# AntonioFerreras/Digital-Earth

Hardware: AMD Instinct MI355X
Metric: Msamples/sec (1920x1080, 64 spp) spectral path tracing (higher is better)
Workload: dtype f32; 1 GPU; 1920x1080, 64 spp, full spectral Rayleigh+Mie+O3+clouds, quality-2 synthetic maps, default camera, BASELINE configs[1]; parallelism=single GPU, frames_in_flight=1, launch_slots=3, waves_per_cu=24, primed_frames=4, kernel=per-CU stage scheduler, launches_per_call=1

## Files before the change

### digital_earth_amd/build.py

```python
import os
import subprocess

_HERE = os.path.dirname(os.path.abspath(__file__))
CSRC = os.path.join(_HERE, "csrc")
OUT = os.path.join(_HERE, "libdigitalearth_hip.so")
OUT_LEGACY = os.path.join(_HERE, "libdigitalearth_hip_legacy.so")
SOURCES = ["de_api.hip", "de_fast.hip"]
DEPS = ["de_api.hip", "de_fast.hip", "de_rccl.h", "de_launch.h", "de_host_consts.h", "de_context.h", "render_kernel.hip", "render_kernel_v2.hip", "de_stages.h", "render_kernel_v6.hip",
        "aux_kernels.hip", "adaptive_kernels.hip", "denoise_kernels.hip", "exposure_kernels.hip", "bloom_kernels.hip", "history_kernels.hip", "pixels_kernels.hip", "local_exposure_kernels.hip", "output_scale_kernels.hip", "hdr_output_kernels.hip", "de_kernels.h", "de_device.h", "de_math.h", os.path.join("..", "..", "include", "digital_earth.h"),
        os.path.join("..", "..", "include", "digital_earth_debug.h"), os.path.join("..", "..", "include", "digital_earth_denoise.h"),
        os.path.join("..", "..", "include", "digital_earth_exposure.h"), os.path.join("..", "..", "include", "digital_earth_bloom.h"),
        os.path.join("..", "..", "include", "digital_earth_history.h"), os.path.join("..", "..", "include", "digital_earth_pixels.h"),
        os.path.join("..", "..", "include", "digital_earth_local_exposure.h"), os.path.join("..", "..", "include", "digital_earth_output_scale.h"),
        os.path.join("..", "..", "include", "digital_earth_hdr_output.h")]
DEPS_LEGACY = DEPS + [os.path.join("legacy", f) for f in ("render_kernel_v3.hip", "render_kernel_v5.hip", "de_launch_legacy.h", "de_ctx_legacy_members.inc")]
FLAGS = ["--offload-arch=gfx950", "-O3", "-std=c++17", "-ffp-contract=off", "-fno-fast-math", "-fno-slp-vectorize", "-fPIC",
         "-shared", "-Wno-unused-value", "-mllvm", "-enable-ipra", "-fno-optimize-sibling-calls"]


def needs_build():
    if not os.path.exists(OUT):
        return True
    t = os.path.getmtime(OUT)
    return any(os.path.getmtime(os.path.join(CSRC, d)) > t for d in DEPS)


def build(force=False, verbose=False):
    if not force and not needs_build():
        return OUT
    hipcc = os.environ.get("HIPCC", "/opt/rocm/bin/hipcc")
    extra = os.environ.get("DE_EXTRA_FLAGS", "").split()
    cmd = [hipcc] + FLAGS + extra + [os.path.join(CSRC, s) for s in SOURCES] + ["-o", OUT]
    if verbose:
        print(" ".join(cmd))
    subprocess.check_call(cmd, cwd=CSRC)
    return OUT


def build_legacy(force=False, verbose=False):
    if not force and os.path.exists(OUT_LEGACY) and all(os.path.getmtime(os.path.join(CSRC, d)) <= os.path.getmtime(OUT_LEGACY) for d in DEPS_LEGACY):
        return OUT_LEGACY
    hipcc = os.environ.get("HIPCC", "/opt/rocm/bin/hipcc")
    cmd = [hipcc] + FLAGS + ["-DDE_LEGACY_VARIANTS"] + os.environ.get("DE_EXTRA_FLAGS", "").split() + [os.path.join(CSRC, s) for s in SOURCES] + ["-o", OUT_LEGACY]
    if verbose:
        print(" ".join(cmd))
    subprocess.check_call(cmd, cwd=CSRC)
    return OUT_LEGACY


TEST_VARIANTS = (("v6_p64", ["-DDE_V6_P=64u", "-DDE_V6_CAP=65u"]), ("v6_p128", ["-DDE_V6_P=128u", "-DDE_V6_CAP=129u"]), ("v6_cap_p1", ["-DDE_V6_CAP=1121u"]),
                 ("v6_no_cloud_bound", ["-DDE_NO_CLOUD_BOUND"]))


def build_test_variants(force=False, verbose=False):
    root = os.path.dirname(_HERE)
    out_dir = os.path.join(root, "build", "ab")
    os.makedirs(out_dir, exist_ok=True)
    hipcc = os.environ.get("HIPCC", "/opt/rocm/bin/hipcc")
    newest = max(os.path.getmtime(os.path.join(CSRC, d)) for d in DEPS)
    procs = []
    for name, flags in TEST_VARIANTS:
        out = os.path.join(out_dir, name + ".so")
        if not force and os.path.exists(out) and os.path.getmtime(out) >= newest:
            continue
        cmd = [hipcc] + FLAGS + flags + [os.path.join(CSRC, s) for s in SOURCES] + ["-o", out]
        if verbose:
            print(" ".join(cmd))
        procs.append((name, subprocess.Popen(cmd, cwd=CSRC)))
    for name, pr in procs:
        if pr.wait() != 0:
            raise RuntimeError("building the test variant %s failed" % name)


if __name__ == "__main__":
    build(force=True, verbose=True)
```

### digital_earth_amd/csrc/de_context.h

```cpp
#pragma once
#include "de_kernels.h"
#include "../../include/digital_earth_exposure.h"
#include "../../include/digital_earth_bloom.h"
#include "../../include/digital_earth_history.h"
#include "../../include/digital_earth_pixels.h"
#include "../../include/digital_earth_local_exposure.h"
#include "../../include/digital_earth_output_scale.h"
#include "../../include/digital_earth_hdr_output.h"

#include <dlfcn.h>
#include <math.h>
#include <stdio.h>
#include <stdlib.h>
#include <string.h>
#include <mutex>
#include <string>
#include <vector>

#include "render_kernel.hip"
#include "render_kernel_v2.hip"
#include "de_stages.h"
#ifdef DE_LEGACY_VARIANTS
#include "legacy/render_kernel_v3.hip"
#include "legacy/render_kernel_v5.hip"
#endif
#include "render_kernel_v6.hip"
#include "aux_kernels.hip"
#include "adaptive_kernels.hip"
#include "denoise_kernels.hip"
#include "exposure_kernels.hip"
#include "bloom_kernels.hip"
#include "history_kernels.hip"
#include "pixels_kernels.hip"
#include "output_scale_kernels.hip"
#include "local_exposure_kernels.hip"
#include "hdr_output_kernels.hip"

namespace {

#define DE_N_COUNTERS 64
thread_local std::string g_err;
int fail(int code, const std::string& msg) { g_err = msg; return code; }

#define HIP_TRY(expr)                                                                                   \
    do {                                                                                                \
        hipError_t e_ = (expr);                                                                         \
        if (e_ != hipSuccess) return fail(DE_ERR_HIP, std::string(#expr) + ": " + hipGetErrorString(e_)); \
    } while (0)

enum { DE_FRAME_NONE = 0, DE_FRAME_UNIFORM = 1, DE_FRAME_ADAPTIVE = 2 };

#define DE_MAX_SLOTS 8
#define DE_FETCH_RING 4
struct LaunchSlot {
    hipStream_t stream = nullptr;
    hipEvent_t done = nullptr;
    hipEvent_t t0 = nullptr, t1 = nullptr;
    uint2* contrib = nullptr;
    size_t contrib_items = 0;
    bool pending = false;
    bool launched = false;
    uint64_t seen_render = 0, seen_hdr = 0;
};

struct DevTexture {
    int w = 0, h = 0, ch = 0;
    uint8_t* linear = nullptr;
    uint32_t* packed = nullptr;
    int tiles_x = 0, tiles_y = 0;
    int packed_clamp = -1;
    uint8_t* bound = nullptr;
    bool set = false;
    bool borrowed = false;
};

}

struct de_ctx {
    int device = 0;
    int W = 0, H = 0;
    de_params p;
    bool params_dirty = true;
    bool nodes_dirty = true;
    int tune_pend = 18, tune_heavy = 13, tune_b = 24, tune_gas = 6, tune_chunk = 128, tune_wpc = 20, tune_max_spp = 0;
    hipStream_t stream = nullptr;
    bool own_stream = false;
    LaunchSlot slot[DE_MAX_SLOTS];
    int n_slots = 8, big_slots = 3, next_slot = 0, last_slot = -1;
    int last_v6_slot = -1;
    int cu_withhold = 0;
    float* d_standin = nullptr;
    hipEvent_t ev_standin[16][2] = {};
    unsigned standin_count = 0;
    bool last_reduce_standin = false;
    hipEvent_t ev_main = nullptr;
    uint64_t gen_render = 1, gen_hdr = 1, rec_render = 0, rec_hdr = 0;
    int t0_slot = -1, t1_slot = -1;
    bool timing_valid = false;
    bool timing_empty = false;
    DevTexture tex[DE_TEX_COUNT];
    float* d_cie = nullptr;
    float* d_srgb2spec = nullptr;
    float* d_o3 = nullptr;
    float* d_crf = nullptr;
    int n_crf = 0;
    bool luts_set = false;
    bool luts_borrowed = false;
    FrameConsts* d_fc = nullptr;
    LambdaNode* d_nodes = nullptr;
    float* d_node_val = nullptr;
    float* d_hdr = nullptr;
    float* d_hdr_own = nullptr;
    float* d_image = nullptr;
    float* d_scratch = nullptr;
    float* h_stage = nullptr;
    size_t h_stage_bytes = 0;
    float* h_ring[DE_FETCH_RING] = {};
    size_t h_ring_bytes[DE_FETCH_RING] = {};
    hipEvent_t ev_ring[DE_FETCH_RING] = {};
    unsigned fetch_begun = 0, fetch_ended = 0;
    uint32_t* d_tiles = nullptr;
    int n_tiles = 0, tiles_rank = -1, tiles_world = -1;
    unsigned long long* d_counters = nullptr;
    uint32_t* d_work_counter = nullptr;
    float* d_dens_table = nullptr;
    int n_cus = 256;
    bool count = false;
    de_counters counters;
    int current_spp = 0;
    int sample_rank = 0, sample_world = 1;
    float* d_assembled = nullptr;
    float* d_gather = nullptr;
    int gather_world = 0;
    const float* display_src = nullptr;
    hipEvent_t ev_r0 = nullptr, ev_r1 = nullptr;
    bool reduce_timing_valid = false;
    void* comm = nullptr;
    int comm_rank = 0, comm_world = 1;
    bool trace = false;
    int kernel_variant = 4;
    struct V6State {
        wf::Cold* cold = nullptr;
        uint32_t* ctl = nullptr;
        RenderArgs* d_args = nullptr;
        uint32_t* h_status = nullptr;
        uint32_t n_wg = 0;
        uint4* pool[2] = {nullptr, nullptr};
        uint32_t pool_cap[2] = {0, 0};
    } v6s[DE_MAX_SLOTS];
    int v6_tail_levels = 1, v6_tail_export[2] = {128, 96}, v6_tail_grid[2] = {64, 8};
    uint32_t v6_tail_min_paths = 4u << 20;
    int v6_tail_when_alone = 0;
    uint32_t* h_issued = nullptr;
    uint32_t v6_launch_seq = 0;
    int v6_bands = 8;
    int v6_stats = 0;
    int v6_svc[3] = {24, 24, 20};
    int v6_svc_area[3] = {100, 72, 90};
    int v6_yield = 56, v6_elsewhere = 48, v6_retry = 6, v6_enter_min = 0, v6_flat_min = 0, v6_flat_again = 32;
    int launch_variant = 2;
    int launch_pipe = 0;
    int launch_slot = 0;
    bool launch_one_batch = false;
    int last_call[4] = {0, 0, 0, 0};
    int launch_pipes = 1;
    int launch_depths = 25, launch_wpc = 14;
    int auto_v6 = 1;
    unsigned long long auto_v6_min_items = 1ull << 12;
    size_t mem_budget = 0;
#ifdef DE_LEGACY_VARIANTS
#include "legacy/de_ctx_legacy_members.inc"
#endif
    int frame_kind = 0;
    float* d_s2 = nullptr;
    uint32_t* d_alist[2] = {nullptr, nullptr};
    int32_t* d_tile_spp = nullptr;
    uint32_t* d_keep = nullptr;
    int32_t* d_ad_count = nullptr;
    int32_t* h_ad_count = nullptr;
    int ad_cur = 0, ad_active = 0, ad_n = 0, ad_rounds = 0;
    unsigned long long ad_pixel_samples = 0;
    uint64_t ad_seed = 0;
    float ad_threshold = 0.f, ad_floor = 0.f;
    int ad_min = 0, ad_max = 0, ad_round = 0;
    bool dn_on = false;
    int dn_levels = 5;
    float dn_sigma_l = 4.0f;
    bool dn_s2_complete = false;
    bool dn_guides_valid = false;
    bool dn_out_valid = false;
    float4* d_dn_nc = nullptr;
    float4* d_dn_at = nullptr;
    float* d_dn_dist = nullptr;
    float4* d_dn_buf[2] = {nullptr, nullptr};
    float* d_dn_out = nullptr;
    bool ae_on = false;
    bool ae_displayed = false;
    de_auto_exposure ae;
    uint32_t* d_ae_partial = nullptr;
    double* d_ae_centre = nullptr;
    MeterState* d_ae_state = nullptr;
    FrameConsts* d_fc_ae = nullptr;
    MeterResult* d_ae_result = nullptr;
    bool bl_on = false;
    de_bloom bl;
    float4* d_bl_pyr = nullptr;
    float* d_bl_out = nullptr;
    bool hs_on = false;
    bool hs_valid = false;
    bool hs_cand_valid = false;
    de_history hs;
    float4* d_hs_c[2] = {nullptr, nullptr};
    float* d_hs_d[2] = {nullptr, nullptr};
    HistoryCam* d_hs_cam[2] = {nullptr, nullptr};
    int hs_cur = 0;
    float* d_hs_out = nullptr;
    de_pixels px = {(uint32_t)sizeof(de_pixels), 4, DE_PIXELS_TRUNCATE, 0u, 0};
    uint32_t px_count = 0;
    uint32_t px_last_phase = 0;
    uint8_t* d_px = nullptr;
    uint8_t* h_px_stage = nullptr;
    uint8_t* h_px_ring[DE_FETCH_RING] = {};
    hipEvent_t ev_px_ring[DE_FETCH_RING] = {};
    unsigned px_begun = 0, px_ended = 0;
    size_t d_px_bytes = 0, h_px_stage_bytes = 0, h_px_ring_bytes[DE_FETCH_RING] = {};
    bool lx_on = false;
    de_local_exposure lx;
    float2* d_lx_pyr = nullptr;
    float* d_lx_base = nullptr;
    float* d_lx_out = nullptr;
    de_output_scale os = {(uint32_t)sizeof(de_output_scale), 0, 0, 0, DE_SCALE_LANCZOS3};
    struct ScaleDev {
        int32_t* first = nullptr;
        float* w = nullptr;
        size_t first_cap = 0, w_cap = 0;
        int n_src = 0, n_dst = 0, filter = -1, taps = 0;
    } os_tab[2];
    float* d_os_mid = nullptr;
    float* d_os_out = nullptr;
    size_t os_mid_bytes = 0, os_out_bytes = 0;
    de_hdr_output ho = {(uint32_t)sizeof(de_hdr_output), 0, 1000.0f, DE_HDR_GAMUT_REC2020, DE_HDR_TRANSFER_PQ, DE_HDR_PIXELS_RGB10A2, DE_PIXELS_TRUNCATE, 0u, 0};
    HdrConsts ho_consts = {};
    uint32_t ho_count = 0;
    uint32_t ho_last_phase = 0;
    void* d_hpx = nullptr;
    uint8_t* h_hpx_stage = nullptr;
    size_t d_hpx_bytes = 0, h_hpx_stage_bytes = 0;
    bool frame_invalid = false;
    std::string invalid_msg;
    de_ctx* lender = nullptr;
    int loans = 0;
};
```

### digital_earth_amd/csrc/de_kernels.h

```cpp
#pragma once
#include "de_device.h"
#include "../../include/digital_earth_debug.h"

struct FrameConsts {
    vec3 cam_pos, d, du, dv;
    float fov, aspect_ratio, aspect_scale;
    vec3 light_dir;
    vec3 sun_x, sun_y;
    float sun_cos_angle, sun_angular_radius;
    float land_height_scale;
    float normal_eps;
    float offset_scale;
    float kn_log;
    float max_dens_r, max_dens_m, max_dens_o;
    CloudPhaseConsts cloud;
    float exposure_scale;
    float gamma;
    float crf_slice_v;
    float vig_strength, vig_radius, vig_cx, vig_cy;
    float drt_m, drt_s, drt_fl, drt_ds, drt_clamp_max, drt_dch_s;
    vec3 drt_w;
    float agx_srgb_to_xyz[9], agx_xyz_to_adjusted[9];
    float agx_x_pivot, agx_y_pivot, agx_toe_scale, agx_shoulder_scale;
    int use_agx;
};

struct LambdaNode {
    float wavelength;
    float rx, ry, rz;
    float rcp_pdf;
    float ext_r, ext_m, ext_o;
    float sun_power, night_power, sun_irradiance;
    float max_ext_rmo;
    float c0, c1, c2;
    float s2s_valid;
    float inv_max_ext_rmo;
    float pad0, pad1, pad2;
};
#define DE_N_NODES 512
#ifndef DE_DENS_TABLE_N
#define DE_DENS_TABLE_N 262144
#endif
#ifndef DE_DENS_STRIDE
#define DE_DENS_STRIDE 3
#endif

struct RenderArgs {
    const FrameConsts* fc;
    const LambdaNode* nodes;
    const float* node_val;
    const float* dens_table;
    TexR8 topo, ocean, clouds, bathy, emissive;
    TexRGB albedo, stars;
    float* hdr;
    int W, H;
    const uint32_t* tiles;
    int n_tiles, tiles_x;
    int tiles_identity;
    uint32_t seed_lo, seed_hi;
    int spp_begin, spp_count;
    int spp_stride;
    int fixed_wavelength;
    unsigned long long* counters;
    float* debug_out;
    uint32_t* work_counter;
    unsigned long long spp_magic;
    uint2* contrib;
    int pend_thr;
    int heavy_thr;
    int chunk;
    int gas_thr;
    int tune_b;
    const uint4* resume_rec;
    const uint32_t* resume_count;
    const float* resume_cold;
    uint32_t resume_capacity;
    const uint8_t* cloud_bound;
};

#ifndef DE_CLOUD_BOUND_N
#define DE_CLOUD_BOUND_N 128
#endif
#ifndef DE_CLOUD_BOUND_R
#define DE_CLOUD_BOUND_R 24576u
#endif
#define DE_CLOUD_BOUND_BYTES (6u * DE_CLOUD_BOUND_N * DE_CLOUD_BOUND_N)
DE_DEV uint32_t cloud_bound_cell(float x, float y, float z) {
    const float ax = de_abs(x), ay = de_abs(y), az = de_abs(z);
    float s, t, m;
    uint32_t f;
    if (ax >= ay && ax >= az) { f = x < 0.0f ? 1u : 0u; s = y; t = z; m = ax; }
    else if (ay >= az) { f = y < 0.0f ? 3u : 2u; s = x; t = z; m = ay; }
    else { f = z < 0.0f ? 5u : 4u; s = x; t = y; m = az; }
    const float r = __builtin_amdgcn_rcpf(m);
    const float hn = (float)(DE_CLOUD_BOUND_N / 2);
    const int i = (int)((s * r + 1.0f) * hn), j = (int)((t * r + 1.0f) * hn);
    const uint32_t ic = (uint32_t)min(max(i, 0), DE_CLOUD_BOUND_N - 1), jc = (uint32_t)min(max(j, 0), DE_CLOUD_BOUND_N - 1);
    return (f * (uint32_t)DE_CLOUD_BOUND_N + jc) * (uint32_t)DE_CLOUD_BOUND_N + ic;
}

struct SetupArgs {
    de_params p;
    int W, H;
    int topo_w;
    int n_crf;
    TexF3 cie;
    const float* srgb2spec;
    const float* o3;
    float drt[6];
    float agx[22];
    FrameConsts* fc;
    LambdaNode* nodes;
    float* node_val;
    int do_nodes;
};

struct DisplayArgs {
    const FrameConsts* fc;
    const float* hdr;
    float* image;
    TexF3 crf;
    int W, H, samples, clamp;
    const int32_t* tile_spp;
};
```

### digital_earth_amd/csrc/de_launch.h

```cpp
#pragma once
#include "de_host_consts.h"

namespace {


int join_slots(de_ctx* c) {
    for (int i = 0; i < c->n_slots; ++i) {
        LaunchSlot& s = c->slot[i];
        if (!s.pending) continue;
        HIP_TRY(hipStreamWaitEvent(c->stream, s.done, 0));
        s.pending = false;
    }
    return DE_OK;
}
bool launches_in_flight(de_ctx* c) {
    bool busy = false;
    for (int i = 0; i < c->n_slots && !busy; ++i)
        if (c->slot[i].launched && hipEventQuery(c->slot[i].done) == hipErrorNotReady) busy = true;
    (void)hipGetLastError();
    return busy;
}
void touched_render_inputs(de_ctx* c) { c->gen_render++; }
void touched_hdr(de_ctx* c) { c->gen_hdr++; }
void note_abort(de_ctx* c);
int frame_status(de_ctx* c);
int sync_all(de_ctx* c) {
    for (int i = 0; i < c->n_slots; ++i)
        if (c->slot[i].stream) HIP_TRY(hipStreamSynchronize(c->slot[i].stream));
    for (int i = 0; i < c->n_slots; ++i) c->slot[i].pending = false;
    HIP_TRY(hipStreamSynchronize(c->stream));
    note_abort(c);
    return DE_OK;
}
void release_loan(de_ctx* c) {
    if (c->lender) { c->lender->loans--; c->lender = nullptr; }
}

int build_cloud_bound(de_ctx* c, DevTexture& t) {
    if (!t.bound) HIP_TRY(hipMalloc(&t.bound, DE_CLOUD_BOUND_BYTES));
    uint8_t* tiles = nullptr;
    HIP_TRY(hipMalloc(&tiles, (size_t)t.tiles_x * t.tiles_y));
    hipLaunchKernelGGL(tile_max_kernel, dim3((unsigned)((t.tiles_x + 255) / 256), (unsigned)t.tiles_y), dim3(256), 0, c->stream, t.packed, tiles, t.w, t.h, t.tiles_x, t.tiles_y);
    hipError_t e = hipGetLastError();
    if (e == hipSuccess) {
        hipLaunchKernelGGL(cloud_bound_kernel, dim3(DE_CLOUD_BOUND_BYTES), dim3(64), 0, c->stream, tiles, t.bound, t.w, t.h, t.tiles_x, t.tiles_y, 1.5 * (double)DE_CLOUD_BOUND_R + 64.0);
        e = hipGetLastError();
    }
    if (e == hipSuccess) e = hipStreamSynchronize(c->stream);
    if (e != hipSuccess) (void)hipStreamSynchronize(c->stream);
    hipFree(tiles);
    if (e != hipSuccess) return fail(DE_ERR_HIP, std::string("building the cloud map's occupancy bound: ") + hipGetErrorString(e));
    return DE_OK;
}

int ensure_packed(de_ctx* c, int slot, bool clamp) {
    DevTexture& t = c->tex[slot];
    if (t.packed_clamp == (clamp ? 1 : 0)) return DE_OK;
    if (t.borrowed) return fail(DE_ERR_STATE, "a shared texture keeps its owner's address mode: set DE_FLAG_CLAMP_SAMPLER on the owner and render there once, then share again");
    if (!t.linear) return fail(DE_ERR_STATE, "the sampler address mode cannot change after de_trim_textures released the as-uploaded maps: upload or generate them again");
    if (c->loans > 0 && t.packed_clamp != -1) return fail(DE_ERR_STATE, "the maps are lent to another context (de_share_textures): they cannot be repacked for another address mode until every borrower is destroyed or holds maps of its own");
    { int rc = join_slots(c); if (rc) return rc; }
    touched_render_inputs(c);
    if (t.ch == 1) {
        dim3 grid((unsigned)((t.w + 255) / 256), (unsigned)t.h);
        hipLaunchKernelGGL(pack_r8_kernel, grid, dim3(256), 0, c->stream, t.linear, t.packed, t.w, t.h, t.tiles_x, clamp ? 1 : 0);
        if (slot == DE_TEX_CLOUDS) { HIP_TRY(hipGetLastError()); int rc = build_cloud_bound(c, t); if (rc) return rc; }
    } else {
        size_t n = (size_t)t.w * t.h;
        hipLaunchKernelGGL(pack_rgb_kernel, dim3((unsigned)((n + 255) / 256)), dim3(256), 0, c->stream, t.linear, t.packed, n);
    }
    HIP_TRY(hipGetLastError());
    t.packed_clamp = clamp ? 1 : 0;
    return DE_OK;
}

int alloc_texture(de_ctx* c, int slot, int w, int h, int ch) {
    DevTexture& t = c->tex[slot];
    if ((unsigned long long)(ch == 1 ? ((w + 7) / 8) * 8 : w) * (unsigned long long)(ch == 1 ? ((h + 3) / 4) * 4 : h) >= (1ull << 30))
        return fail(DE_ERR_INVALID, "map too large: the packed copy (one dword per texel) must stay below 4 GB — the kernels address it with a 32-bit byte offset");
    if (c->loans > 0) return fail(DE_ERR_STATE, "the maps are lent to another context (de_share_textures): destroy the borrowers, or give them maps of their own, before replacing a map");
    { int rc = sync_all(c); if (rc) return rc; }
    if (t.linear && !t.borrowed) hipFree(t.linear);
    if (t.packed && !t.borrowed) hipFree(t.packed);
    if (t.bound && !t.borrowed) hipFree(t.bound);
    t.linear = nullptr; t.packed = nullptr; t.bound = nullptr; t.borrowed = false;
    {
        bool any = false;
        for (int i = 0; i < DE_TEX_COUNT; ++i) any = any || (i != slot && c->tex[i].borrowed);
        if (!any && !c->luts_borrowed) release_loan(c);
    }
    touched_render_inputs(c);
    t.w = w; t.h = h; t.ch = ch; t.set = false; t.packed_clamp = -1;
    HIP_TRY(hipMalloc(&t.linear, (size_t)w * h * ch));
    if (ch == 1) {
        t.tiles_x = (w + 7) / 8; t.tiles_y = (h + 3) / 4;
        HIP_TRY(hipMalloc(&t.packed, (size_t)t.tiles_x * t.tiles_y * 32 * sizeof(uint32_t)));
    } else {
        t.tiles_x = t.tiles_y = 0;
        HIP_TRY(hipMalloc(&t.packed, (size_t)w * h * sizeof(uint32_t)));
    }
    return DE_OK;
}

int run_setup(de_ctx* c) {
    if (!c->params_dirty && !c->nodes_dirty) return DE_OK;
    { int rc = join_slots(c); if (rc) return rc; }
    touched_render_inputs(c);
    SetupArgs s;
    s.p = c->p;
    opendrt_consts(&s.drt[0], &s.drt[1], &s.drt[2], &s.drt[3], &s.drt[4], &s.drt[5]);
    agx_consts(s.agx);
    s.W = c->W; s.H = c->H;
    s.topo_w = c->tex[DE_TEX_TOPOGRAPHY].w > 0 ? c->tex[DE_TEX_TOPOGRAPHY].w : 1;
    s.n_crf = c->n_crf;
    s.cie.data = c->d_cie; s.cie.w = 441; s.cie.h = 2;
    s.srgb2spec = c->d_srgb2spec; s.o3 = c->d_o3;
    s.fc = c->d_fc; s.nodes = c->d_nodes; s.node_val = c->d_node_val;
    s.do_nodes = c->nodes_dirty ? 1 : 0;
    hipLaunchKernelGGL(setup_kernel, dim3(c->nodes_dirty ? DE_N_NODES / 64 : 1), dim3(64), 0, c->stream, s);
    HIP_TRY(hipGetLastError());
    c->params_dirty = false; c->nodes_dirty = false;
    return DE_OK;
}

int build_tiles(de_ctx* c, int rank, int world) {
    if (c->tiles_rank == rank && c->tiles_world == world && c->d_tiles) return DE_OK;
    { int rc = sync_all(c); if (rc) return rc; }
    touched_render_inputs(c);
    const int tx = c->W / 8, ty = c->H / 8;
    std::vector<uint32_t> tiles;
    tiles.reserve((size_t)tx * ty / world + tx);
    for (int y = 0; y < ty; ++y)
        for (int x = 0; x < tx; ++x)
            if (world <= 1 || ((x + y) % world) == rank) tiles.push_back((uint32_t)(y * tx + x));
    if (!c->d_tiles) HIP_TRY(hipMalloc(&c->d_tiles, (size_t)tx * ty * sizeof(uint32_t)));
    if (!tiles.empty()) HIP_TRY(hipMemcpyAsync(c->d_tiles, tiles.data(), tiles.size() * sizeof(uint32_t), hipMemcpyHostToDevice, c->stream));
    HIP_TRY(hipStreamSynchronize(c->stream));
    c->n_tiles = (int)tiles.size(); c->tiles_rank = rank; c->tiles_world = world;
    return DE_OK;
}

int fill_render_args(de_ctx* c, RenderArgs* a) {
    for (int i = 0; i < DE_TEX_COUNT; ++i)
        if (!c->tex[i].set) return fail(DE_ERR_STATE, "all 7 textures must be uploaded or generated before rendering");
    if (!c->luts_set) return fail(DE_ERR_STATE, "LUTs must be uploaded before rendering");
    const bool clamp = (c->p.flags & DE_FLAG_CLAMP_SAMPLER) != 0;
    for (int i = 0; i < DE_TEX_COUNT; ++i) { int rc = ensure_packed(c, i, clamp); if (rc) return rc; }
    int rc = run_setup(c);
    if (rc) return rc;
    auto r8 = [&](int slot) {
        const DevTexture& t = c->tex[slot];
        TexR8 o; o.data = t.packed; o.w = t.w; o.h = t.h; o.tiles_x = t.tiles_x; o.wf = (float)t.w; o.hf = (float)t.h;
        return o;
    };
    auto rgb = [&](int slot) {
        const DevTexture& t = c->tex[slot];
        TexRGB o; o.data = t.packed; o.w = t.w; o.h = t.h; o.wf = (float)t.w; o.hf = (float)t.h;
        return o;
    };
    a->fc = c->d_fc; a->nodes = c->d_nodes; a->node_val = c->d_node_val; a->dens_table = c->d_dens_table;
    a->topo = r8(DE_TEX_TOPOGRAPHY); a->ocean = r8(DE_TEX_OCEAN); a->clouds = r8(DE_TEX_CLOUDS);
    a->bathy = r8(DE_TEX_BATHYMETRY); a->emissive = r8(DE_TEX_EMISSIVE);
    a->albedo = rgb(DE_TEX_ALBEDO); a->stars = rgb(DE_TEX_STARS);
    a->hdr = c->d_hdr; a->W = c->W; a->H = c->H;
    a->tiles = c->d_tiles; a->n_tiles = c->n_tiles; a->tiles_x = c->W / 8; a->tiles_identity = (c->tiles_world <= 1) ? 1 : 0;
    a->fixed_wavelength = (c->p.flags & DE_FLAG_FIXED_WAVELENGTH) ? 1 : 0;
    a->counters = c->d_counters; a->debug_out = c->d_scratch; a->work_counter = c->d_work_counter;
    a->resume_rec = nullptr; a->resume_count = nullptr; a->resume_cold = nullptr; a->resume_capacity = 0;
    a->cloud_bound = c->tex[DE_TEX_CLOUDS].bound;
    a->pend_thr = c->tune_pend; a->heavy_thr = c->tune_heavy; a->tune_b = c->tune_b; a->gas_thr = c->tune_gas; a->chunk = c->tune_chunk;
    return DE_OK;
}

#ifdef DE_LEGACY_VARIANTS
hipError_t launch_v3(de_ctx* c, const RenderArgs& a, hipStream_t stream, int pipe);
hipError_t launch_v5(de_ctx* c, const RenderArgs& a, hipStream_t stream, int idx, const uint4* resume_rec = nullptr, const uint32_t* resume_count = nullptr,
                     const float* resume_cold = nullptr, uint32_t resume_capacity = 0, int wpc = 0);
void legacy_note_abort(de_ctx* c);
#endif

int v6_reserve(de_ctx* c, int idx, hipStream_t stream, unsigned long long n_items) {
    de_ctx::V6State& S = c->v6s[idx];
    const uint32_t n_wg = (uint32_t)(c->cu_withhold > 0 ? c->n_cus - 8 * c->cu_withhold : c->n_cus) * DE_V6_WG_PER_CU;
    uint32_t want[2] = {0u, 0u};
    const bool tail = n_items >= (unsigned long long)c->v6_tail_min_paths;
    if (tail && c->v6_tail_levels >= 1) want[0] = n_wg * (uint32_t)c->v6_tail_export[0];
    if (tail && c->v6_tail_levels >= 2) want[1] = std::min((uint32_t)c->v6_tail_grid[0], n_wg) * (uint32_t)c->v6_tail_export[1];
    for (int k = 0; k < 2; ++k) {
        if (S.pool_cap[k] >= want[k]) continue;
        HIP_TRY(hipStreamSynchronize(stream));
        if (S.pool[k]) hipFree(S.pool[k]);
        S.pool[k] = nullptr; S.pool_cap[k] = 0;
        if (hipMalloc(&S.pool[k], (size_t)want[k] * DE_V6_POOL_ENTRY_BYTES + 64u) != hipSuccess) { (void)hipGetLastError(); S.pool[k] = nullptr; return fail(DE_ERR_NOMEM, "no room for the tail pool of a render_kernel_v6 launch slot"); }
        S.pool_cap[k] = want[k];
    }
    if (S.cold && S.ctl && S.d_args && S.h_status && S.n_wg == n_wg) return DE_OK;
    HIP_TRY(hipStreamSynchronize(stream));
    if (S.cold) hipFree(S.cold);
    S.cold = nullptr; S.n_wg = 0;
    if (hipMalloc(&S.cold, (size_t)n_wg * DE_V6_P * sizeof(wf::Cold)) != hipSuccess) { (void)hipGetLastError(); S.cold = nullptr; return fail(DE_ERR_NOMEM, "no room for the cold records of a render_kernel_v6 launch slot (37 MB)"); }
    S.n_wg = n_wg;
    if (!S.ctl) HIP_TRY(hipMalloc(&S.ctl, (size_t)bs::G_WORDS * DE_V6_CTL_STRIDE * sizeof(uint32_t)));
    if (!S.d_args) HIP_TRY(hipMalloc(&S.d_args, sizeof(RenderArgs)));
    if (!S.h_status) {
        HIP_TRY(hipHostMalloc(reinterpret_cast<void**>(&S.h_status), 64, hipHostMallocMapped));
        S.h_status[0] = 0u;
    }
    return DE_OK;
}
}
hipError_t de_fast_launch_v6(const bs::Args& A, const FrameConsts* fc, dim3 grid, dim3 block, hipStream_t stream, bool clamp, bool tail);
namespace {
hipError_t launch_v6(de_ctx* c, const RenderArgs& a, hipStream_t stream, int idx) {
    de_ctx::V6State& S = c->v6s[idx];
    const bool clamp = (c->p.flags & DE_FLAG_CLAMP_SAMPLER) != 0;
    bs::Args A;
    A.ra = S.d_args; A.cold = S.cold; A.ctl = S.ctl;
    uint32_t* d_status = nullptr;
    hipError_t e = hipHostGetDevicePointer(reinterpret_cast<void**>(&d_status), S.h_status, 0);
    if (e != hipSuccess) return e;
    A.status = d_status;
    A.n_items = (uint32_t)((size_t)a.n_tiles * 64u * (size_t)a.spp_count);
    A.idle_limit = 1u << 22;
    for (int k = 0; k < 3; ++k) { A.svc[k] = (uint32_t)c->v6_svc[k]; A.svc_area[k] = (uint32_t)c->v6_svc_area[k]; }
    A.yield_max = (uint32_t)c->v6_yield; A.elsewhere_min = (uint32_t)c->v6_elsewhere; A.retry = (uint32_t)c->v6_retry; A.enter_min = (uint32_t)c->v6_enter_min; A.flat_min = (uint32_t)c->v6_flat_min; A.flat_again = (uint32_t)(c->v6_flat_again > 0 ? c->v6_flat_again : 1);
    A.bands = c->v6_bands == 8 ? 8u : 1u;
    hipLaunchKernelGGL(v6_init_kernel, dim3(1), dim3(256), 0, stream, S.ctl, a, S.d_args);
    const unsigned by_work = (unsigned)((A.n_items + 64u * DE_V6_WAVES - 1u) / (64u * DE_V6_WAVES));
    dim3 grid(by_work < S.n_wg ? (by_work ? by_work : 1u) : S.n_wg), block(64 * DE_V6_WAVES);
    const int levels = A.n_items >= c->v6_tail_min_paths ? c->v6_tail_levels : 0;
    if (!c->h_issued) {
        e = hipHostMalloc(reinterpret_cast<void**>(&c->h_issued), 64, hipHostMallocMapped);
        if (e != hipSuccess) return e;
        c->h_issued[0] = 0u;
    }
    uint32_t* d_issued = nullptr;
    e = hipHostGetDevicePointer(reinterpret_cast<void**>(&d_issued), c->h_issued, 0);
    if (e != hipSuccess) return e;
    const uint32_t seq = ++c->v6_launch_seq;
    if (c->last_v6_slot >= 0 && c->last_v6_slot != idx) __atomic_store_n(c->h_issued, seq - 1u, __ATOMIC_RELEASE);
    c->last_v6_slot = idx;
    A.issued = d_issued; A.seq = c->v6_tail_when_alone ? 0xffffffffu : seq;
    const bool fast = (c->p.flags & DE_FLAG_FAST_MATH) != 0u;
    for (int l = 0; l <= levels; ++l) {
        A.level = (uint32_t)l;
        A.export_at = l < levels ? (uint32_t)c->v6_tail_export[l] : 0u;
        A.pool_out = l < levels ? S.pool[l & 1] : nullptr; A.cap_out = l < levels ? S.pool_cap[l & 1] : 0u;
        A.pool_in = l > 0 ? S.pool[(l - 1) & 1] : nullptr; A.cap_in = l > 0 ? S.pool_cap[(l - 1) & 1] : 0u;
        const dim3 g = l == 0 ? grid : dim3(std::min((unsigned)c->v6_tail_grid[l - 1], (unsigned)S.n_wg));
        if (fast) { hipError_t e2 = de_fast_launch_v6(A, a.fc, g, block, stream, clamp, l > 0); if (e2 != hipSuccess) return e2; continue; }
        if (l == 0) {
            if (c->v6_stats && !clamp) hipLaunchKernelGGL((v6_kernel<false, true, false>), g, block, 0, stream, A, a.fc);
            else if (clamp) hipLaunchKernelGGL((v6_kernel<true, false, false>), g, block, 0, stream, A, a.fc);
            else hipLaunchKernelGGL((v6_kernel<false, false, false>), g, block, 0, stream, A, a.fc);
        } else {
            if (c->v6_stats && !clamp) hipLaunchKernelGGL((v6_kernel<false, true, true>), g, block, 0, stream, A, a.fc);
            else if (clamp) hipLaunchKernelGGL((v6_kernel<true, false, true>), g, block, 0, stream, A, a.fc);
            else hipLaunchKernelGGL((v6_kernel<false, false, true>), g, block, 0, stream, A, a.fc);
        }
    }
    return hipGetLastError();
}
void note_abort(de_ctx* c) {
    for (int i = 0; i < DE_MAX_SLOTS; ++i) {
        de_ctx::V6State& S = c->v6s[i];
        if (S.h_status && S.h_status[0] != 0u) {
            const uint32_t code = S.h_status[0];
            S.h_status[0] = 0u;
            c->frame_invalid = true;
            c->invalid_msg = std::string("render_kernel_v6 left on its abort word (") + (code == bs::ERR_ENTRY_TIMEOUT ? "a ring entry was never stored" : code == bs::ERR_CELL_BUSY_TIMEOUT ? "a ring cell was never emptied" : code == bs::ERR_POOL_FULL ? "the tail pool overflowed" : "idle watchdog: work was lost") + "): the frame is invalid until de_reset";
        }
    }
#ifdef DE_LEGACY_VARIANTS
    legacy_note_abort(c);
#endif
}
int frame_status(de_ctx* c) {
    note_abort(c);
    return c->frame_invalid ? fail(DE_ERR_HIP, c->invalid_msg) : DE_OK;
}

hipError_t launch_accumulate(de_ctx* c, const RenderArgs& a, dim3 grid, dim3 block, hipStream_t stream) {
    if (c->frame_kind == DE_FRAME_ADAPTIVE || (c->dn_on && c->dn_s2_complete)) hipLaunchKernelGGL(accumulate_moments_kernel, grid, block, 0, stream, a, c->d_s2);
    else hipLaunchKernelGGL(accumulate_kernel, grid, block, 0, stream, a);
    return hipGetLastError();
}

template <int MODE, typename PreAcc>
hipError_t launch_render(de_ctx* c, const RenderArgs& a, hipStream_t stream, PreAcc pre_acc) {
    const bool clamp = (c->p.flags & DE_FLAG_CLAMP_SAMPLER) != 0;
    const bool march = (c->p.flags & DE_FLAG_RAY_MARCHER) != 0;
    dim3 grid((unsigned)((a.n_tiles + 3) / 4)), block(256);
#ifdef DE_LEGACY_VARIANTS
    if (!march && (c->launch_variant == 5 || c->launch_variant == 3) && MODE == 0) {
        hipError_t el = c->launch_variant == 5 ? launch_v5(c, a, stream, c->launch_slot) : launch_v3(c, a, stream, c->launch_pipe);
        if (el != hipSuccess) return el;
        hipError_t pe = pre_acc();
        if (pe != hipSuccess) return pe;
        return launch_accumulate(c, a, grid, block, stream);
    }
#endif
    if (!march && c->launch_variant == 6 && MODE == 0) {
        hipError_t e6 = launch_v6(c, a, stream, c->launch_slot);
        if (e6 != hipSuccess) return e6;
        hipError_t pe = pre_acc();
        if (pe != hipSuccess) return pe;
        return launch_accumulate(c, a, grid, block, stream);
    }
    if (!march && c->launch_variant != 1) {
        hipError_t me = hipMemsetAsync(a.work_counter, 0, sizeof(uint32_t), stream);
        if (me != hipSuccess) return me;
        const unsigned waves_per_block = DE_V2_BLOCK / 64;
        const unsigned waves_per_cu = (unsigned)c->tune_wpc;
        const unsigned max_waves = (unsigned)c->n_cus * waves_per_cu;
        const unsigned long long items = (unsigned long long)a.n_tiles * 64ull * (unsigned long long)a.spp_count;
        const unsigned long long by_work = (items + (unsigned long long)a.chunk - 1ull) / (unsigned long long)a.chunk;
        const unsigned n_waves = by_work >= (unsigned long long)max_waves ? max_waves : (unsigned)(by_work > 0 ? by_work : 1ull);
        dim3 pgrid((n_waves + waves_per_block - 1) / waves_per_block), pblock(DE_V2_BLOCK);
        if (clamp) hipLaunchKernelGGL((render_kernel_v2<true, MODE>), pgrid, pblock, 0, stream, a, a.fc);
        else hipLaunchKernelGGL((render_kernel_v2<false, MODE>), pgrid, pblock, 0, stream, a, a.fc);
        if (MODE != 2) {
            hipError_t pe = pre_acc();
            if (pe != hipSuccess) return pe;
            return launch_accumulate(c, a, grid, block, stream);
        }
        return hipGetLastError();
    }
    hipError_t pe = pre_acc();
    if (pe != hipSuccess) return pe;
    if (march) {
        if (clamp) hipLaunchKernelGGL((ray_march_kernel<true, MODE>), grid, block, 0, stream, a);
        else hipLaunchKernelGGL((ray_march_kernel<false, MODE>), grid, block, 0, stream, a);
    }
#ifdef DE_LEGACY_VARIANTS
    else if (clamp) hipLaunchKernelGGL((render_kernel<true, false, MODE>), grid, block, 0, stream, a);
    else hipLaunchKernelGGL((render_kernel<false, false, MODE>), grid, block, 0, stream, a);
#endif
    return hipGetLastError();
}

hipError_t stage_ensure(de_ctx* c, size_t bytes) {
    if (c->h_stage && c->h_stage_bytes < bytes) { (void)hipHostFree(c->h_stage); c->h_stage = nullptr; c->h_stage_bytes = 0; }
    if (c->h_stage) return hipSuccess;
    hipError_t e = hipHostMalloc((void**)&c->h_stage, bytes, hipHostMallocDefault);
    if (e != hipSuccess) { c->h_stage = nullptr; (void)hipGetLastError(); return e; }
    c->h_stage_bytes = bytes;
    return hipSuccess;
}

int copy_out(de_ctx* c, float* out, const float* d_src, size_t bytes = 0) {
    if (!bytes) bytes = (size_t)c->W * c->H * 3 * sizeof(float);
    (void)stage_ensure(c, bytes);
    if (c->h_stage) {
        HIP_TRY(hipMemcpyAsync(c->h_stage, d_src, bytes, hipMemcpyDeviceToHost, c->stream));
        HIP_TRY(hipStreamSynchronize(c->stream));
        memcpy(out, c->h_stage, bytes);
    } else {
        HIP_TRY(hipMemcpyAsync(out, d_src, bytes, hipMemcpyDeviceToHost, c->stream));
        HIP_TRY(hipStreamSynchronize(c->stream));
    }
    return frame_status(c);
}

int accumulate_default(de_ctx* c, RenderArgs& a, int spp, int first_index) {
    const bool march = (c->p.flags & DE_FLAG_RAY_MARCHER) != 0;
    const bool records = !march;
    const unsigned long long call_items = (unsigned long long)a.n_tiles * 64ull * (unsigned long long)(spp > 0 ? spp : 0);
    const bool fast = (c->p.flags & DE_FLAG_FAST_MATH) != 0u;
    const bool v6k = records && !c->count && (fast || c->kernel_variant == 6 || (c->kernel_variant == 4 && call_items >= c->auto_v6_min_items));
    int max_spp = spp > 0 ? spp : 1;
    if (records && a.n_tiles > 0) {
        const unsigned long long nt = (unsigned long long)a.n_tiles;
        unsigned long long cap = ((1ull << 29) / (nt * 64ull));
        while (cap > 1 && nt * cap * cap >= (1ull << 40)) --cap;
        if (cap < 1) cap = 1;
        if (c->tune_max_spp > 0 && cap > (unsigned long long)c->tune_max_spp) cap = (unsigned long long)c->tune_max_spp;
        if ((unsigned long long)max_spp > cap) max_spp = (int)cap;
        if (max_spp < spp) { const int nl = (spp + max_spp - 1) / max_spp; max_spp = (spp + nl - 1) / nl; }
        if (nt * 64ull * (unsigned long long)max_spp >= (1ull << 32) || nt * (unsigned long long)max_spp * (unsigned long long)max_spp >= (1ull << 40))
            return fail(DE_ERR_INVALID, "image too large for the 32-bit work-item index of a launch");
    }
    if (c->rec_render != c->gen_render || c->rec_hdr != c->gen_hdr) {
        HIP_TRY(hipEventRecord(c->ev_main, c->stream));
        c->rec_render = c->gen_render; c->rec_hdr = c->gen_hdr;
    }
    bool first = true;
    c->last_call[0] = 0; c->last_call[1] = 1; c->last_call[2] = 0; c->last_call[3] = 0;
    c->timing_empty = true;
    for (int done = 0; done < spp && a.n_tiles > 0;) {
        const int n = (spp - done < max_spp) ? spp - done : max_spp;
        const size_t need = records ? (size_t)a.n_tiles * 64u * (size_t)n : 0;
        const int n_want = (need * sizeof(uint2) > ((size_t)96 << 20)) ? (c->big_slots < c->n_slots ? c->big_slots : c->n_slots) : c->n_slots;
        const int n_cycle = n_want < c->n_slots ? n_want : c->n_slots;
        const int si = c->next_slot % n_cycle;
        c->launch_slot = si;
        LaunchSlot& s = c->slot[si];
        if (v6k) { int rc6 = v6_reserve(c, si, s.stream, (unsigned long long)a.n_tiles * 64ull * (unsigned long long)n); if (rc6) return rc6; }
        c->launch_variant = v6k ? 6 : 2;
        if (need > s.contrib_items) {
            for (int j = 0; j < n_cycle; ++j) {
                LaunchSlot& sj = c->slot[j];
                if (need <= sj.contrib_items) continue;
                HIP_TRY(hipStreamSynchronize(sj.stream));
                if (sj.contrib) hipFree(sj.contrib);
                sj.contrib = nullptr; sj.contrib_items = 0;
                if (hipMalloc(&sj.contrib, need * sizeof(uint2)) != hipSuccess) { (void)hipGetLastError(); return fail(DE_ERR_NOMEM, "no room for the per-sample records of a launch (8 bytes per path)"); }
                sj.contrib_items = need;
            }
        }
        a.contrib = s.contrib;
        a.work_counter = c->d_work_counter + 16 * si;
        a.spp_begin = first_index + done * a.spp_stride; a.spp_count = n;
        a.spp_magic = ((1ull << 40) / (unsigned long long)n) + 1ull;
        if (s.seen_render != c->gen_render) {
            HIP_TRY(hipStreamWaitEvent(s.stream, c->ev_main, 0));
            s.seen_render = c->gen_render; s.seen_hdr = c->gen_hdr;
        }
        if (first) { HIP_TRY(hipEventRecord(s.t0, s.stream)); c->t0_slot = si; first = false; }
        const int prev = c->last_slot;
        auto pre_acc = [&]() -> hipError_t {
            if (s.seen_hdr != c->gen_hdr) {
                hipError_t e = hipStreamWaitEvent(s.stream, c->ev_main, 0);
                if (e != hipSuccess) return e;
                s.seen_hdr = c->gen_hdr;
            }
            if (prev >= 0 && prev != si) return hipStreamWaitEvent(s.stream, c->slot[prev].done, 0);
            return hipSuccess;
        };
        HIP_TRY(c->count ? launch_render<1>(c, a, s.stream, pre_acc) : launch_render<0>(c, a, s.stream, pre_acc));
        c->last_call[0] = march ? 0 : c->launch_variant;
        c->last_call[3]++;
        HIP_TRY(hipEventRecord(s.done, s.stream));
        s.pending = true; s.launched = true;
        c->last_slot = si;
        c->next_slot = (si + 1) % n_cycle;
        done += n;
        if (done >= spp) { HIP_TRY(hipEventRecord(s.t1, s.stream)); c->t1_slot = si; c->timing_valid = true; c->timing_empty = false; }
    }
    return DE_OK;
}

}

#ifdef DE_LEGACY_VARIANTS
#include "legacy/de_launch_legacy.h"
#endif
```

### digital_earth_amd/csrc/de_stages.h

```cpp
#pragma once
#include "de_kernels.h"
#include "render_kernel_v2.hip"

namespace wf {

template <typename T> DE_DEV const T* opaque_ptr(const T* p) {
    uint32_t lo = (uint32_t)__builtin_amdgcn_readfirstlane((int)(uint32_t)(uintptr_t)p), hi = (uint32_t)__builtin_amdgcn_readfirstlane((int)(uint32_t)((uintptr_t)p >> 32));
    asm volatile("" : "+s"(lo), "+s"(hi));
    return reinterpret_cast<const T*>((uintptr_t)lo | ((uintptr_t)hi << 32));
}

enum { Q_ST = 0, Q_GAS, Q_CLOUD, Q_EVENT, Q_SURF, Q_SCFIN, Q_SURFFIN, NQ };
enum { EV_NULL = 0, EV_ABSORB = 1, EV_SCATTER = 2 };

struct Cold { float thr, Ls, dx, dy, dz, nx, ny, nz, alb, ocean, bathy, pad0, pad1, pad2, pad3, pad4; };

struct Path {
    uint32_t pid, meta;
    Rng rng;
    vec3 P, W;
    float x[6];
};
DE_DEV int m_kind(uint32_t m) { return (int)(m & 3u); }
DE_DEV int m_node(uint32_t m) { return (int)((m >> 2) & 511u); }
DE_DEV int m_sc(uint32_t m) { return (int)((m >> 11) & 31u); }
DE_DEV int m_below(uint32_t m) { return (int)((m >> 16) & 1u); }
DE_DEV int m_evid(uint32_t m) { return (int)((m >> 17) & 7u); }
DE_DEV int m_event(uint32_t m) { return (int)((m >> 20) & 63u); }
DE_DEV uint32_t m_make(int kind, int node, int sc, int below, int ev_id, int event) {
    return (uint32_t)kind | ((uint32_t)node << 2) | ((uint32_t)sc << 11) | ((uint32_t)below << 16) | ((uint32_t)ev_id << 17) | ((uint32_t)event << 20);
}
DE_DEV float asf(uint32_t u) { return __builtin_bit_cast(float, u); }
DE_DEV uint32_t asu(float f) { return __builtin_bit_cast(uint32_t, f); }

DE_DEV void cloud_limits_of_ray(vec3 ray_pos, vec3 ray_dir, float* t_start_out, float* t_max_out, int* below_out) {
    v2::cloud_limits_of_ray(ray_pos, ray_dir, t_start_out, t_max_out, below_out);
}

DE_DEV int enter_cloud(Path& p, float c_ts, float c_tm, float aux, float X) {
    const int kind = m_kind(p.meta);
    const float t_start = c_ts;
    const float t_max = (m_below(p.meta) && X > 0.0f) ? -1.0f : c_tm;
    bool run = true;
    if (kind == 0) run = ((m_event(p.meta) & 15) == EV_NULL) || (aux > t_start);
    const bool enter = run && (t_start < t_max);
    if (enter) { p.x[0] = t_start; p.x[1] = t_max; p.x[2] = aux; p.x[3] = X; return Q_CLOUD; }
    if (kind == 0) { p.x[0] = t_start; p.x[1] = aux; p.x[2] = X; return Q_EVENT; }
    p.x[0] = aux; p.x[1] = 1.0f; p.x[2] = X;
    return kind == 1 ? Q_SCFIN : Q_SURFFIN;
}
DE_DEV int after_sphere_trace(Path& p, float t, float max_ray_dist) {
    const int kind = m_kind(p.meta);
    const float atm_x = p.x[1], atm_y = p.x[2], c_ts = p.x[3], c_tm = p.x[4];
    const float hit = (t < max_ray_dist) ? t : -1.0f;
    const float X = (kind == 0) ? hit : ((hit < 0.0f) ? -1.0f : 0.0f);
    const float t_start = de_max(0.0f, atm_x);
    float t_max = (X >= 0.0f) ? X : atm_y;
    if (atm_y < 0.0f) t_max = -1.0f;
    if (t_start < t_max) { p.x[0] = t_start; p.x[1] = t_max; p.x[2] = c_ts; p.x[3] = c_tm; p.x[4] = X; return Q_GAS; }
    return enter_cloud(p, c_ts, c_tm, (kind == 0) ? t_start : 1.0f, X);
}
DE_DEV void ray_head(Path& p) {
    const vec2_ atmos = rsi(p.P, p.W, DE_ATMOS_UPPER);
    float c_ts, c_tm; int below;
    cloud_limits_of_ray(p.P, p.W, &c_ts, &c_tm, &below);
    p.x[0] = (atmos.x > 0.0f) ? atmos.x : 0.0f;
    p.x[1] = atmos.x; p.x[2] = atmos.y; p.x[3] = c_ts; p.x[4] = c_tm;
    p.meta = (p.meta & ~(1u << 16)) | ((uint32_t)below << 16);
}

template <bool CLAMP>
DE_DEV float sphere_trace(const RenderArgs& a, const Path& p, float land_height_scale, float escape_r, float max_ray_dist) {
    float t = p.x[0];
    int cnt = 0;
    for (;;) {
        const vec3 Q = p.P + p.W * t;
        const float len = length_nr(Q);
        if (cnt <= 100) {
            const float b = dot(Q, p.W);
            const float peri2 = (b < 0.0f) ? (len * len - b * b) : len * len;
            if (peri2 > escape_r * escape_r) { t = max_ray_dist; break; }
        }
        const vec3 n = Q * de_rcp_nr(len);
        const vec2_ uv = sphere_UV_map(n);
        const float tex = tap_r8<CLAMP>(a.topo, fract_(uv.x * 1.0f), fract_(uv.y * 1.0f));
        const float sdf = len - DE_PLANET_R - land_height_scale * tex;
        t += sdf;
        cnt++;
        if (t > max_ray_dist || de_abs(sdf) < t * 0.0001f || cnt >= 250) break;
    }
    return t;
}

DE_DEV void write_contrib(const RenderArgs& a, uint32_t pid, float Ls, int node) {
    if (__builtin_isinf(Ls) || Ls != Ls || Ls < 0.0f) Ls = 0.0f;
    a.contrib[pid] = make_uint2(asu(Ls), (uint32_t)node);
}


DE_DEV void new_path(const RenderArgs& a, const FrameConsts& fc, const float* s_node_val, uint32_t w, Path& p) {
    const uint32_t wq = w >> 6;
    const uint32_t tile_k = (uint32_t)(((unsigned long long)wq * a.spp_magic) >> 40);
    const uint32_t tile = a.tiles_identity ? tile_k : a.tiles[tile_k];
    const int s_idx = (int)(wq - tile_k * (uint32_t)a.spp_count);
    const int sub = (int)(w & 63u);
    const int u = (int)(tile % (uint32_t)a.tiles_x) * 8 + (sub & 7);
    const int v = (int)(tile / (uint32_t)a.tiles_x) * 8 + (sub >> 3);
    const uint32_t pixel = (uint32_t)(v * a.W + u);
    rng_seed(p.rng, a.seed_lo, a.seed_hi, pixel, (uint32_t)(a.spp_begin + s_idx * a.spp_stride));
    int node = 0;
    if (!a.fixed_wavelength) {
        const float sample = rng_next(p.rng);
        node = 1;
#pragma unroll
        for (int it = 0; it < 8; ++it) {
            const float val = (it < 6) ? s_node_val[node] : a.node_val[node];
            if (val < sample) node = 2 * node + 1;
            else if (val > sample) node = 2 * node;
            else break;
        }
    }
    p.pid = w;
    p.W = v2::get_cast_dir(p.rng, fc, a.H, u, v);
    p.P = fc.cam_pos;
    p.meta = m_make(0, node, 0, 0, 0, 0);
    p.x[5] = 0.0f;
    ray_head(p);
}


template <bool CLAMP, typename ColdT>
DE_DEV int event_body(const RenderArgs& a, const FrameConsts& fc, const ColdT& cold, Path& p) {
    int target = -1;
    const int sc = m_sc(p.meta), node = m_node(p.meta);
    const int rmo_event = m_event(p.meta);
    const int cloud_event = rmo_event >> 4, gas_event = rmo_event & 15;
    const float t = p.x[0], rmo_t = p.x[1], isect = p.x[2];
    const vec3 D = p.W;
    int event = gas_event;
    float tt = rmo_t;
    int id = m_evid(p.meta);
    if (cloud_event > 0 && (t < rmo_t || gas_event == EV_NULL)) { tt = t; id = CLOUD_ID; event = cloud_event; }
    if (sc > 9 && id == CLOUD_ID) id = ISOTROPIC_CLOUD_ID;
    vec3 LD;
    {
        const vec3 cv = sample_cone(p.rng, fc.sun_cos_angle);
        const vec3 bx = fc.sun_x, by = fc.sun_y, bn = fc.light_dir;
        LD = v3((bx.x * cv.x + by.x * cv.y) + bn.x * cv.z, (bx.y * cv.x + by.y * cv.y) + bn.y * cv.z, (bx.z * cv.x + by.z * cv.y) + bn.z * cv.z);
    }
    bool end = false, miss = false;
    if (event == EV_ABSORB) {
        end = true;
    } else if (event == EV_SCATTER) {
        p.P = p.P + tt * D;
        if (sc == 0) cold.set_thr_ls(p.pid, 1.0f, 0.0f);
        cold.set_dir(p.pid, D);
        p.W = LD;
        const bool blocked = rsi(p.P, LD, DE_PLANET_R).y > 0.0f;
        if (blocked) {
            p.meta = m_make(1, node, sc, 0, id, 0);
            p.x[0] = 0.0f; p.x[1] = 1.0f; p.x[2] = 1.0f;
            target = Q_SCFIN;
        } else {
            const vec2_ atmos = rsi(p.P, LD, DE_ATMOS_UPPER);
            float c_ts, c_tm; int below;
            cloud_limits_of_ray(p.P, LD, &c_ts, &c_tm, &below);
            p.meta = m_make(1, node, sc, below, id, 0);
            const float t_start = de_max(0.0f, atmos.x);
            float t_max = atmos.y;
            if (atmos.y < 0.0f) t_max = -1.0f;
            if (t_start < t_max) {
                p.x[0] = t_start; p.x[1] = t_max; p.x[2] = c_ts; p.x[3] = c_tm; p.x[4] = -1.0f;
                target = Q_GAS;
            } else {
                target = enter_cloud(p, c_ts, c_tm, 1.0f, -1.0f);
            }
        }
    } else if (isect > 0.0f) {
        p.P = p.P + D * isect;
        if (sc == 0) cold.set_thr_ls(p.pid, 1.0f, 0.0f);
        cold.set_dir(p.pid, D);
        p.W = LD;
        p.meta = m_make(2, node, sc, 0, id, 0);
        target = Q_SURF;
    } else {
        end = true;
        miss = (sc == 0);
    }
    if (end) {
        const LambdaNode& L = a.nodes[node];
        float Ls = (sc == 0) ? 0.0f : cold.get_ls(p.pid);
        if (miss) {
            if (dot(fc.light_dir, D) > fc.sun_cos_angle) Ls += L.sun_power;
            const vec3 stars_srgb = sphere_tap_rgb<CLAMP>(a.stars, normalized(D));
            const float stars_power = v2::srgb_to_spectrum(L, stars_srgb);
            Ls += stars_power * L.sun_power * 0.0000001f;
        }
        write_contrib(a, p.pid, Ls, node);
    }
    return target;
}

template <bool CLAMP, typename ColdT>
DE_DEV int surf_body(const RenderArgs& a, const FrameConsts& fc, const ColdT& cold, Path& p) {
    const float land_height_scale = fc.land_height_scale, e = fc.normal_eps;
    const LambdaNode& L = a.nodes[m_node(p.meta)];
    auto sdf_at = [&](vec3 Q) -> float {
        const float len = length_nr(Q);
        const vec3 nn = Q * de_rcp_nr(len);
        const vec2_ uv = sphere_UV_map(nn);
        const float tex = tap_r8<CLAMP>(a.topo, fract_(uv.x * 1.0f), fract_(uv.y * 1.0f));
        return len - DE_PLANET_R - land_height_scale * tex;
    };
    const float d0 = sdf_at(p.P);
    vec3 N = v3(d0 - sdf_at(p.P - v3(e, 0.0f, 0.0f)), d0 - sdf_at(p.P - v3(0.0f, e, 0.0f)), d0 - sdf_at(p.P - v3(0.0f, 0.0f, e)));
    N = normalized(N);
    const vec3 nrm = normalized(p.P);
    const vec2_ uv = sphere_UV_map(nrm);
    const float uu = fract_(uv.x * 1.0f), vv = fract_(uv.y * 1.0f);
    const float ocean = tap_r8<CLAMP>(a.ocean, uu, vv);
    const vec3 tex = tap_rgb<CLAMP>(a.albedo, uu, vv);
    vec3 land = mix3(lum3(tex), tex, 6.5f);
    float greenery = sqr(land.y / lum(land));
    greenery = smoothstep_(1.5f, 1.9f, greenery);
    land = (1.0f * tex) / (greenery * 0.7f + 1.0f);
    land = mix3(lum3(land), land, 1.4f - greenery * 0.45f);
    land = mix3(land, (land * v3(255.0f, 128.0f, 64.0f)) / 255.0f, 0.2f * (1.0f - greenery));
    const vec3 ocean_albedo = mix3(lum3(tex), tex, 0.75f) * 0.9f;
    const vec3 albedo_srgb = mix3(land, ocean_albedo, ocean);
    const float bathy = tap_r8<CLAMP>(a.bathy, uu, vv);
    const float emissive = tap_r8<CLAMP>(a.emissive, uu, vv);
    const float alb = v2::srgb_to_spectrum(L, albedo_srgb);
    float thr, Ls;
    cold.get_thr_ls(p.pid, thr, Ls);
    cold.set_thr_ls(p.pid, thr, Ls + thr * emissive * L.night_power);
    cold.set_surf(p.pid, N, alb, ocean, bathy);
    p.P = p.P * fc.offset_scale;
    ray_head(p);
    return Q_ST;
}

template <typename ColdT>
DE_DEV int vertex_end(const RenderArgs& a, const ColdT& cold, Path& p, int node, int sc, float thr, float Ls, vec3 nd) {
    bool end = false;
    if (sc > 3) {
        const float termination_p = de_max(0.05f, 1.0f - thr);
        if (rng_next(p.rng) < termination_p) end = true;
        else thr /= 1.0f - termination_p;
    }
    sc++;
    if (!end && sc >= 25) end = true;
    if (end) {
        write_contrib(a, p.pid, Ls, node);
        return -1;
    }
    cold.set_thr_ls(p.pid, thr, Ls);
    p.W = nd;
    p.meta = m_make(0, node, sc, 0, 0, 0);
    ray_head(p);
    return Q_ST;
}

template <typename ColdT>
DE_DEV int scfin_body(const RenderArgs& a, const FrameConsts& fc, const ColdT& cold, Path& p) {
    const int node = m_node(p.meta), ev_id = m_evid(p.meta);
    const int sc = m_sc(p.meta);
    const LambdaNode& L = a.nodes[node];
    float thr, Ls;
    cold.get_thr_ls(p.pid, thr, Ls);
    const vec3 D = cold.get_dir(p.pid), LD = p.W;
    const float trg = p.x[0], trn = p.x[1], li = p.x[2];
    const float direct_tr = (li > 0.0f) ? 0.0f : trg * trn;
    const float direct_phase = v2::evaluate_phase(fc, D, LD, ev_id, sc > 0);
    Ls += thr * direct_tr * L.sun_irradiance * direct_phase;
    float phase_div_pdf;
    const vec3 nd = v2::sample_phase(fc, p.rng, D, ev_id, sc > 0, &phase_div_pdf);
    thr *= phase_div_pdf;
    return vertex_end(a, cold, p, node, sc, thr, Ls, nd);
}

template <typename ColdT>
DE_DEV int surffin_body(const RenderArgs& a, const ColdT& cold, Path& p) {
    const int node = m_node(p.meta);
    const int sc = m_sc(p.meta);
    const LambdaNode& L = a.nodes[node];
    float thr, Ls;
    cold.get_thr_ls(p.pid, thr, Ls);
    const vec3 D = cold.get_dir(p.pid), LD = p.W;
    vec3 N; float alb, ocean, bathy;
    cold.get_surf(p.pid, N, alb, ocean, bathy);
    const float trg = p.x[0], trn = p.x[1], li = p.x[2];
    const float direct_tr = trg * trn;
    const bool visible = li < 0.0f;
    float direct_ndl;
    const float direct_brdf = earth_brdf(alb, ocean, bathy, -D, N, LD, &direct_ndl);
    Ls += thr * direct_tr * (visible ? 1.0f : 0.0f) * L.sun_irradiance * direct_brdf * direct_ndl;
    const vec3 view_dir = -D;
    const vec3 nd = sample_hemisphere_cosine_weighted(p.rng, N);
    float unused;
    const float brdf = earth_brdf(alb, ocean, bathy, view_dir, N, nd, &unused);
    thr *= brdf * (float)M_PI;
    return vertex_end(a, cold, p, node, sc, thr, Ls, nd);
}

}

template <bool CLAMP>
struct StStage {
    const TexR8 topo;
    float land_height_scale, escape_r, max_ray_dist;
    float t; int cnt;
    DE_DEV void begin(wf::Path& p) { t = p.x[0]; cnt = 0; }
    struct Tok { uint32_t q; float fx, fy, len; };
    DE_DEV bool issue(wf::Path& p, Tok& k) {
        const vec3 Q = p.P + p.W * t;
        const float len = length_nr(Q);
        if (cnt <= 100) {
            const float b = dot(Q, p.W);
            const float peri2 = (b < 0.0f) ? (len * len - b * b) : len * len;
            if (peri2 > escape_r * escape_r) { t = max_ray_dist; return true; }
        }
        const vec3 n = Q * de_rcp_nr(len);
        const vec2_ uv = sphere_UV_map(n);
        k.q = tap_r8_issue<CLAMP>(topo, fract_(uv.x * 1.0f), fract_(uv.y * 1.0f), &k.fx, &k.fy);
        k.len = len;
        return false;
    }
    DE_DEV bool resolve(wf::Path&, const Tok& k) {
        const float tex = tap_r8_finish(k.q, k.fx, k.fy);
        const float sdf = k.len - DE_PLANET_R - land_height_scale * tex;
        t += sdf;
        cnt++;
        return t > max_ray_dist || de_abs(sdf) < t * 0.0001f || cnt >= 250;
    }
    DE_DEV bool step(wf::Path& p) { Tok k; return issue(p, k) || resolve(p, k); }
    DE_DEV int finish(wf::Path& p) { return wf::after_sphere_trace(p, t, max_ray_dist); }
    DE_DEV void suspend(wf::Path& p, wf::Cold* c) const { p.x[0] = t; c->pad1 = wf::asf((uint32_t)cnt); }
    DE_DEV void restore(const wf::Cold* c) { cnt = (int)wf::asu(c->pad1); }
};

struct GasStage {
    const LambdaNode* nodes;
    const float* dens_table;
    float ext_r, ext_m, ext_o, rmaxr, t, tmax, trn;
    vec3 C;
    int kind, event, ev_id;
    DE_DEV void begin(wf::Path& p) {
        const LambdaNode& L = nodes[wf::m_node(p.meta)];
        ext_r = L.ext_r; ext_m = L.ext_m; ext_o = L.ext_o; rmaxr = L.inv_max_ext_rmo;
        kind = wf::m_kind(p.meta);
        t = p.x[0]; tmax = p.x[1];
        C = p.P + t * p.W;
        trn = 1.0f; event = wf::EV_NULL; ev_id = 0;
    }
    DE_DEV bool step(wf::Path& p) {
        const float neg_log = -de_log_unit(rng_next(p.rng));
        const float t_step = neg_log * rmaxr;
        C = C + t_step * p.W;
        t += t_step;
        if (t >= tmax) return true;
        const float len = length_nr(C);
        const float h2 = de_max(len - DE_PLANET_R, 0.0f) * 2.0f;
        vec3 dens;
#ifndef DE_GAS_TABLE
        (void)h2;
        dens = get_density(de_max(len - DE_PLANET_R, 0.0f));
#else
        if (h2 < (float)DE_DENS_TABLE_N) {
            dens = dens_table_read(dens_table, (uint32_t)(int)h2);
        } else {
            dens = get_density(len - DE_PLANET_R);
        }
#endif
        const vec3 es = v3(ext_r, ext_m, ext_o) * dens;
        const float sum = (es.x + es.y) + es.z;
        const float pr = sum * rmaxr;
        const bool delta = kind == 0;
        Rng g = p.rng;
        const float rand = rng_next(g);
        p.rng.s0 = delta ? g.s0 : p.rng.s0; p.rng.s1 = delta ? g.s1 : p.rng.s1;
        const float trn_r = trn * (1.0f - pr);
        trn = delta ? trn : trn_r;
        bool done = !delta & (trn_r < 1e-5f);
        if (delta & (rand < pr)) {
            int id = 0;
            float cmf = es.x;
            if (!(rand < cmf * rmaxr)) {
                id = 1;
                cmf += es.y;
                if (!(rand < cmf * rmaxr)) {
                    id = 2;
                    cmf += es.z;
                    if (!(rand < cmf * rmaxr)) id = 3;
                }
            }
            const float albedo = (id == 0) ? 1.0f : ((id == 1) ? 0.95f : ((id == 2) ? 0.0f : 0.99f));
            event = (rng_next(p.rng) < albedo) ? wf::EV_SCATTER : wf::EV_ABSORB;
            ev_id = id;
            done = true;
        }
        return done | !(t < tmax);
    }
    DE_DEV int finish(wf::Path& p) {
        if (kind == 0) p.meta = (p.meta & ~((7u << 17) | (63u << 20))) | ((uint32_t)ev_id << 17) | ((uint32_t)event << 20);
        return wf::enter_cloud(p, p.x[2], p.x[3], (kind == 0) ? t : trn, p.x[4]);
    }
    DE_DEV void suspend(wf::Path& p, wf::Cold* c) const { p.x[0] = t; c->pad1 = trn; c->pad2 = C.x; c->pad3 = C.y; c->pad4 = C.z; }
    DE_DEV void restore(const wf::Cold* c) { trn = c->pad1; C = v3(c->pad2, c->pad3, c->pad4); }
};

template <bool CLAMP, bool BOUND = false>
struct CloudStage {
    static constexpr bool kBound = BOUND;
    const TexR8 clouds;
    const uint8_t* bound;
    float ext_w, rmaxc, t, tmax, trn;
    vec3 C;
    int kind, cloud_event;
#ifndef DE_NO_TAP_REUSE
    uint32_t last_idx = 0xffffffffu, last_q = 0u;
#endif
    uint32_t bnd = 0xffffffffu;
    bool exact = true, looked = false;
    DE_DEV void begin(wf::Path& p) {
        const int sc = wf::m_sc(p.meta);
        ext_w = (sc > 9) ? 0.02f : DE_CLOUDS_EXTINCT;
        rmaxc = (sc > 9) ? (1.0f / (0.02f * DE_CLOUDS_DENSITY)) : (1.0f / (DE_CLOUDS_EXTINCT * DE_CLOUDS_DENSITY));
        kind = wf::m_kind(p.meta);
        t = p.x[0]; tmax = p.x[1];
        C = p.P + t * p.W;
        trn = 1.0f; cloud_event = 0;
        bnd = 0xffffffffu;
    }
    struct Tok { uint32_t q; float fx, fy, h; bool shell; };
    DE_DEV bool issue(wf::Path& p, Tok& k) {
        exact = false; looked = false;
        const float neg_log = -de_log_unit(rng_next(p.rng));
        const float t_step = neg_log * rmaxc;
        C = C + t_step * p.W;
        t += t_step;
        if (t >= tmax) return true;
        const float len = length_nr(C);
        k.shell = len > DE_CLOUDS_LOWER && len < DE_CLOUDS_UPPER;
        k.h = (len - DE_CLOUDS_LOWER) * (1.0f / DE_CLOUDS_THICKNESS);
        exact = k.shell;
        if (BOUND) {
            if (k.shell) {
                bnd -= ((uint32_t)t_step + 1u) << 8;
                if ((int32_t)bnd < 0) {
                    const uint32_t cell = cloud_bound_cell(C.x, C.y, C.z);
                    typedef const __attribute__((address_space(1))) uint8_t* de_gbytes;
                    bnd = (uint32_t)*((de_gbytes)bound + cell) | (DE_CLOUD_BOUND_R << 8);
                    looked = true;
                }
                const float T = (float)(bnd & 255u) * DE_INV_255;
                const float split = 0.2f;
                k.shell = (k.h - split < T * (float)(1.0 - 0.2)) & (split - k.h < T * split);
            } else {
                bnd = 0xffffffffu;
            }
            exact = k.shell;
        }
        if (k.shell) {
            const vec3 nrm = C * de_rcp_nr(len);
            const vec2_ uv = sphere_UV_map(nrm);
#ifndef DE_NO_TAP_REUSE
            k.q = tap_r8_issue_cached<CLAMP>(clouds, fract_(uv.x * 1.0f), fract_(uv.y * 1.0f), &k.fx, &k.fy, last_idx, last_q);
#else
            k.q = tap_r8_issue<CLAMP>(clouds, fract_(uv.x * 1.0f), fract_(uv.y * 1.0f), &k.fx, &k.fy);
#endif
        }
        return false;
    }
    DE_DEV bool resolve(wf::Path& p, const Tok& k) {
        float density = 0.0f;
        if (k.shell) {
            const float tex = tap_r8_finish(k.q, k.fx, k.fy);
            const float h = k.h;
            const float split = 0.2f;
            density = ((h - split < tex * (float)(1.0 - 0.2)) & (split - h < tex * split)) ? de_max(tex, 0.4f) : 0.0f;
        }
        const float es = ext_w * (density * DE_CLOUDS_DENSITY);
        const float pr = es * rmaxc;
        const bool delta = kind == 0;
        Rng g = p.rng;
        const float rand = rng_next(g);
        p.rng.s0 = delta ? g.s0 : p.rng.s0; p.rng.s1 = delta ? g.s1 : p.rng.s1;
        const float trn_r = trn * (1.0f - pr);
        trn = delta ? trn : trn_r;
        bool done = !delta & (trn_r < 1e-5f);
        if (delta & (rand < pr)) { cloud_event = (rng_next(p.rng) < 0.99f) ? wf::EV_SCATTER : wf::EV_ABSORB; done = true; }
        return done | !(t < tmax);
    }
    DE_DEV bool step(wf::Path& p) { Tok k; return issue(p, k) || resolve(p, k); }
    DE_DEV int finish(wf::Path& p) {
        const float aux = p.x[2], X = p.x[3];
        if (kind == 0) {
            p.meta |= ((uint32_t)cloud_event << 4) << 20;
            p.x[0] = t; p.x[1] = aux; p.x[2] = X;
            return wf::Q_EVENT;
        }
        p.x[0] = aux; p.x[1] = trn; p.x[2] = X;
        return (kind == 1) ? wf::Q_SCFIN : wf::Q_SURFFIN;
    }
    DE_DEV void suspend(wf::Path& p, wf::Cold* c) const { p.x[0] = t; c->pad1 = trn; c->pad2 = C.x; c->pad3 = C.y; c->pad4 = C.z; }
    DE_DEV void restore(const wf::Cold* c) { trn = c->pad1; C = v3(c->pad2, c->pad3, c->pad4); bnd = 0xffffffffu; }
};
```

### digital_earth_amd/csrc/render_kernel_v6.hip

```cpp
#include "de_stages.h"

namespace bs {

using wf::Path;
using wf::NQ;
using wf::Q_ST; using wf::Q_GAS; using wf::Q_CLOUD; using wf::Q_EVENT; using wf::Q_SURF; using wf::Q_SCFIN; using wf::Q_SURFFIN;

enum { Q_FREE = NQ, NR = NQ + 1, Q_PRIMARY = NQ + 1, Q_EXIT = NQ + 2, Q_EXPORT = NQ + 3 };
#ifndef DE_V6_WAVES
#define DE_V6_WAVES 12
#endif
#ifndef DE_V6_WG_PER_CU
#define DE_V6_WG_PER_CU 2
#endif
#ifndef DE_V6_WPE
#define DE_V6_WPE 6
#endif
#ifndef DE_V6_P
#define DE_V6_P 1120u
#endif
#ifndef DE_V6_CAP
#define DE_V6_CAP 1128u
#endif
#define DE_V6_EMPTY 0xffffu
#define DE_V6_SLOT_MASK 0x7ffu
static_assert(DE_V6_P < DE_V6_SLOT_MASK, "slot numbers take 11 bits of a ring cell; the all-ones pattern marks an empty cell");
static_assert(DE_V6_CAP >= DE_V6_P, "a ring must be able to hold every slot number");
static_assert(DE_V6_WAVES <= 31, "the lap tag of a ring cell has five bits: one open lap per blocked wave at most");
#define DE_V6_CTL_STRIDE 32u
enum { G_WORK = 0, G_T_START = 1, G_T_EXHAUSTED = 2, G_T_END = 3, G_STAT0 = 8, G_STAT2 = 8 + 64, G_WORKX = 8 + 64 + 64, G_DRAIN = 8 + 64 + 64 + 8, G_POOL = 8 + 64 + 64 + 8 + 64, G_WORDS = 8 + 64 + 64 + 8 + 64 + 8 };
enum { R_STEP = 0, R_EPI, R_PUSH, R_REFILL, R_YIELD, R_HEAD, R_N };
enum { ST_RECS = 0, ST_CYC = 8, ST_IDLE = 16, ST_ENTRIES = 17, ST_CLAIMFAIL = 18, ST_SCHED = 19, ST_YIELD = 20, ST_YIELDED = 21, ST_DRAIN = 22, ST_CLOUD_EXACT = 23, ST_ENTRY_Q = 24, ST_CLOUD_NOEXACT = 31, ST_TRIPS = 32, ST_CLOUD_LOOKUPS = 39, ST_LANETRIPS = 40, ST_N = 48 };
enum { ERR_ENTRY_TIMEOUT = 1, ERR_CELL_BUSY_TIMEOUT = 2, ERR_IDLE_WATCHDOG = 3, ERR_POOL_FULL = 4 };
DE_DEV uint32_t cell_empty(uint32_t lap) { return (lap << 11) | DE_V6_SLOT_MASK; }
DE_DEV uint32_t cell_full(uint32_t lap, uint32_t slot) { return (lap << 11) | slot; }
DE_DEV uint32_t cell_for(uint32_t v, uint32_t lap) { return (v ^ (lap << 11)) & 0xffffu; }

struct Args {
    const RenderArgs* ra;
    wf::Cold* cold;
    uint32_t* ctl;
    uint32_t* status;
    uint32_t n_items;
    uint32_t idle_limit;
    uint32_t svc[3];
    uint32_t svc_area[3];
    uint32_t yield_max;
    uint32_t elsewhere_min;
    uint32_t retry;
    uint32_t enter_min;
    uint32_t flat_min;
    uint32_t flat_again;
    uint32_t bands;
    uint32_t level;
    uint32_t export_at;
    uint4* pool_in; uint4* pool_out;
    uint32_t cap_in, cap_out;
    const uint32_t* issued;
    uint32_t seq;
};
template <int... T> struct Targets {};

struct Pool {
    uint4 *a, *b, *c, *cold; uint2* d; uint32_t* q;
    DE_DEV Pool(uint4* base, uint32_t cap) : a(base), b(base + cap), c(base + 2u * cap), cold(base + 3u * cap), d(reinterpret_cast<uint2*>(base + 7u * (size_t)cap)), q(reinterpret_cast<uint32_t*>(base + 7u * (size_t)cap) + 2u * (size_t)cap) {}
};
#define DE_V6_POOL_ENTRY_BYTES 124u

struct Cfg {
    const RenderArgs* ra;
    const FrameConsts* fc;
    wf::Cold* cold;
    uint32_t* ctl;
    uint32_t* status;
    uint32_t n_items, idle_limit;
    uint32_t svc[3];
    uint32_t svc_area[3];
    uint32_t yield_max, elsewhere_min, retry, enter_min;
    uint32_t flat_min, flat_again;
    uint32_t bands, xcd;
    uint4* pool_in; uint4* pool_out;
    const uint32_t* issued;
    uint32_t level, export_at, cap_in, cap_out, seq, pad_;
};
static_assert(sizeof(Cfg) % 4 == 0 && sizeof(Cfg) <= 160, "Cfg is copied dword by dword");

__shared__ uint4 s_rec[3u * DE_V6_P];
__shared__ uint2 s_rec2[DE_V6_P];
__shared__ uint16_t s_rings[(NQ + 1) * DE_V6_CAP];
__shared__ uint32_t s_cw[32];
__shared__ float s_node_val[64];
__shared__ unsigned long long s_stats[64];
__shared__ uint32_t s_cfg[40];

DE_DEV int lane_id() { return (int)__builtin_amdgcn_mbcnt_hi(~0u, __builtin_amdgcn_mbcnt_lo(~0u, 0u)); }
DE_DEV uint32_t uni(uint32_t v) { return (uint32_t)__builtin_amdgcn_readfirstlane((int)v); }
DE_DEV float unif(float v) { return __builtin_bit_cast(float, __builtin_amdgcn_readfirstlane(__builtin_bit_cast(int, v))); }
template <typename T>
DE_DEV const T* uni_ptr(const T* p) {
    const unsigned long long u = (unsigned long long)p;
    const unsigned long long lo = (uint32_t)__builtin_amdgcn_readfirstlane((int)(uint32_t)u), hi = (uint32_t)__builtin_amdgcn_readfirstlane((int)(uint32_t)(u >> 32));
    return reinterpret_cast<const T*>((hi << 32) | lo);
}
DE_DEV TexR8 uni_tex(const TexR8& t) {
    TexR8 o;
    o.data = uni_ptr(t.data);
    o.w = __builtin_amdgcn_readfirstlane(t.w); o.h = __builtin_amdgcn_readfirstlane(t.h); o.tiles_x = __builtin_amdgcn_readfirstlane(t.tiles_x);
    o.wf = unif(t.wf); o.hf = unif(t.hf);
    return o;
}
DE_DEV uint32_t ld_wg(const uint32_t* p) { return __hip_atomic_load(p, __ATOMIC_RELAXED, __HIP_MEMORY_SCOPE_WORKGROUP); }
DE_DEV uint32_t add_wg(uint32_t* p, uint32_t v) { return __hip_atomic_fetch_add(p, v, __ATOMIC_RELAXED, __HIP_MEMORY_SCOPE_WORKGROUP); }
DE_DEV uint32_t ld_e(const uint16_t* p) { return (uint32_t)__hip_atomic_load(p, __ATOMIC_RELAXED, __HIP_MEMORY_SCOPE_WORKGROUP); }
DE_DEV void st_e(uint16_t* p, uint32_t v) { __hip_atomic_store(p, (uint16_t)v, __ATOMIC_RELAXED, __HIP_MEMORY_SCOPE_WORKGROUP); }
DE_DEV void release_wg() { __builtin_amdgcn_fence(__ATOMIC_RELEASE, "workgroup"); }
DE_DEV void acquire_wg() { __builtin_amdgcn_fence(__ATOMIC_ACQUIRE, "workgroup"); }

DE_DEV void load_rec(const uint4* rec, uint32_t s, Path& p) {
    const uint4 a = rec[s], b = rec[DE_V6_P + s], c = rec[2u * DE_V6_P + s];
    const uint2 d = s_rec2[s];
    p.pid = 0u; p.meta = a.x; p.rng.s0 = a.y; p.rng.s1 = a.z; p.rng.draws = 0;
    p.P = v3(wf::asf(a.w), wf::asf(b.x), wf::asf(b.y)); p.W = v3(wf::asf(b.z), wf::asf(b.w), wf::asf(c.x));
    p.x[0] = wf::asf(c.y); p.x[1] = wf::asf(c.z); p.x[2] = wf::asf(c.w); p.x[3] = wf::asf(d.x); p.x[4] = wf::asf(d.y); p.x[5] = 0.0f;
}
DE_DEV void store_rec(uint4* rec, uint32_t s, const Path& p) {
    rec[s] = make_uint4(p.meta, p.rng.s0, p.rng.s1, wf::asu(p.P.x));
    rec[DE_V6_P + s] = make_uint4(wf::asu(p.P.y), wf::asu(p.P.z), wf::asu(p.W.x), wf::asu(p.W.y));
    rec[2u * DE_V6_P + s] = make_uint4(wf::asu(p.W.z), wf::asu(p.x[0]), wf::asu(p.x[1]), wf::asu(p.x[2]));
    s_rec2[s] = make_uint2(wf::asu(p.x[3]), wf::asu(p.x[4]));
}

struct ColdAt {
    wf::Cold* c;
    DE_DEV void get_thr_ls(uint32_t, float& thr, float& Ls) const { thr = c->thr; Ls = c->Ls; }
    DE_DEV float get_ls(uint32_t) const { return c->Ls; }
    DE_DEV void set_thr_ls(uint32_t, float thr, float Ls) const { c->thr = thr; c->Ls = Ls; }
    DE_DEV vec3 get_dir(uint32_t) const { return v3(c->dx, c->dy, c->dz); }
    DE_DEV void set_dir(uint32_t, vec3 D) const { c->dx = D.x; c->dy = D.y; c->dz = D.z; }
    DE_DEV void set_surf(uint32_t, vec3 N, float alb, float ocean, float bathy) const { c->nx = N.x; c->ny = N.y; c->nz = N.z; c->alb = alb; c->ocean = ocean; c->bathy = bathy; }
    DE_DEV void get_surf(uint32_t, vec3& N, float& alb, float& ocean, float& bathy) const { N = v3(c->nx, c->ny, c->nz); alb = c->alb; ocean = c->ocean; bathy = c->bathy; }
};

template <bool CLAMP, bool STATS>
struct Wave {
    Cfg A;
    uint4* rec;
    uint16_t* rings;
    uint32_t* cw;
    wf::Cold* cold;
    unsigned long long* s_st;
    bool primary_left, aborted;
    unsigned long long t_mark;
    unsigned long long r_t[R_N], r_l[R_N], r_last, r_cnt[2];

    DE_DEV void regions_begin() {
        if (!STATS) return;
#pragma unroll
        for (int k = 0; k < R_N; ++k) { r_t[k] = 0ull; r_l[k] = 0ull; }
        r_cnt[0] = r_cnt[1] = 0ull;
        r_last = __builtin_amdgcn_s_memtime();
    }
    template <int R>
    DE_DEV void tick(unsigned long long lanes) {
        if (!STATS) return;
        const unsigned long long t = __builtin_amdgcn_s_memtime(), dt = t - r_last;
        r_t[R] += dt; r_l[R] += dt * lanes; r_last = t;
    }
    DE_DEV void stat2(int k, unsigned long long v) {
        if (STATS && lane_id() == 0 && v) __hip_atomic_fetch_add(reinterpret_cast<unsigned long long*>(A.ctl + (G_STAT2 + k) * DE_V6_CTL_STRIDE), v, __ATOMIC_RELAXED, __HIP_MEMORY_SCOPE_AGENT);
    }
    DE_DEV void regions_end_loop(int q) {
        if (!STATS) return;
#pragma unroll
        for (int k = 0; k < R_N; ++k) { stat2(14 * q + 2 * k, r_t[k]); stat2(14 * q + 2 * k + 1, r_l[k]); }
        stat2(14 * q + 12, r_cnt[0]); stat2(14 * q + 13, r_cnt[1]);
    }
    DE_DEV void regions_end_flat(int base) {
        if (!STATS) return;
        stat2(base, r_t[R_STEP]); stat2(base + 1, r_l[R_STEP]); stat2(base + 2, r_t[R_PUSH]); stat2(base + 3, r_cnt[0]);
    }

    DE_DEV static Wave enter() {
        Wave W;
        uint32_t* dst = reinterpret_cast<uint32_t*>(&W.A);
#pragma unroll
        for (uint32_t k = 0; k < sizeof(Cfg) / 4u; ++k) dst[k] = uni(s_cfg[k]);
        W.rec = s_rec; W.rings = s_rings; W.cw = s_cw; W.cold = W.A.cold; W.s_st = s_stats;
        W.primary_left = true; W.aborted = false; W.t_mark = 0ull;
        return W;
    }

    template <typename Stage>
    DE_DEV void cloud_stats(const Stage& st, bool stepping) {
        if constexpr (Stage::kBound) {
            const unsigned long long n_exact = (unsigned long long)__popcll(__ballot(stepping && st.exact));
            stat(ST_CLOUD_EXACT, n_exact);
            stat(ST_CLOUD_NOEXACT, n_exact == 0ull && __ballot(stepping) != 0ull ? 1ull : 0ull);
            stat(ST_CLOUD_LOOKUPS, (unsigned long long)__popcll(__ballot(stepping && st.looked)));
        }
    }
    DE_DEV void stat(int k, unsigned long long v) { if (STATS && lane_id() == 0) __hip_atomic_fetch_add(s_st + k, v, __ATOMIC_RELAXED, __HIP_MEMORY_SCOPE_WORKGROUP); }
    template <int STAGE>
    DE_DEV void mark() {
        if (!STATS) return;
        const unsigned long long t = __builtin_amdgcn_s_memrealtime();
        stat(STAGE >= 0 ? ST_CYC + STAGE : ST_SCHED, t - t_mark);
        t_mark = t;
    }
    DE_DEV uint32_t* head(uint32_t q) const { return cw + q; }
    DE_DEV uint32_t* tail(uint32_t q) const { return cw + 8u + q; }
    DE_DEV void raise(uint32_t code) {
        if (lane_id() == 0) {
            __hip_atomic_store(cw + 16, code, __ATOMIC_RELAXED, __HIP_MEMORY_SCOPE_WORKGROUP);
            __hip_atomic_store(A.status, code, __ATOMIC_RELAXED, __HIP_MEMORY_SCOPE_SYSTEM);
        }
        aborted = true;
    }

    DE_DEV bool starters() { primary_left = uni(ld_wg(cw + 19)) < A.bands; return primary_left; }

    DE_DEV uint32_t claim(uint32_t q, uint32_t kmin, uint32_t kmax, uint32_t* first) {
        uint32_t got = 0, hh = 0;
        if (lane_id() == 0) {
            uint32_t h = ld_wg(head(q));
#pragma nounroll
            for (int tries = 0; tries < 16; ++tries) {
                const uint32_t t = ld_wg(tail(q));
                const int avail = (int)(t - h);
                if (avail < (int)kmin) break;
                const uint32_t k = (uint32_t)avail < kmax ? (uint32_t)avail : kmax;
                uint32_t expected = h;
                if (__hip_atomic_compare_exchange_strong(head(q), &expected, h + k, __ATOMIC_RELAXED, __ATOMIC_RELAXED, __HIP_MEMORY_SCOPE_WORKGROUP)) { got = k; hh = h; break; }
                h = expected;
            }
        }
        *first = uni(hh);
        return uni(got);
    }
    __device__ __attribute__((noinline)) uint32_t wait_cell(uint16_t* e, uint32_t lap, bool want_entry) {
        uint32_t x = DE_V6_SLOT_MASK + 1u;
#pragma nounroll
        for (uint32_t spins = 0; spins < (1u << 20); ++spins) {
            x = cell_for(ld_e(e), lap);
            if (want_entry ? x < DE_V6_SLOT_MASK : x == DE_V6_SLOT_MASK) return x;
            __builtin_amdgcn_s_sleep(1);
        }
        return DE_V6_SLOT_MASK + 1u;
    }
    DE_DEV uint32_t take(uint32_t q, uint32_t idx) {
        const uint32_t lap = idx / DE_V6_CAP;
        uint16_t* e = rings + q * DE_V6_CAP + (idx - lap * DE_V6_CAP);
        uint32_t x = cell_for(ld_e(e), lap);
        if (__ballot(x >= DE_V6_SLOT_MASK) != 0ull) {
            if (x >= DE_V6_SLOT_MASK) x = wait_cell(e, lap, true);
            if (x >= DE_V6_SLOT_MASK) return DE_V6_EMPTY;
        }
        st_e(e, cell_empty(lap + 1u));
        return x;
    }
    template <int Q>
    DE_DEV void push(uint32_t slot, bool pred) {
        const unsigned long long mask = __ballot(pred);
        if (mask == 0ull) return;
        const uint32_t n = (uint32_t)__popcll(mask), rank = (uint32_t)__popcll(mask & ((1ull << lane_id()) - 1ull));
        uint32_t base = 0;
        if (lane_id() == 0) base = add_wg(tail(Q), n);
        base = uni(base);
        if (pred) {
            const uint32_t idx = base + rank, lap = idx / DE_V6_CAP;
            uint16_t* e = rings + Q * DE_V6_CAP + (idx - lap * DE_V6_CAP);
            bool ok = cell_for(ld_e(e), lap) == DE_V6_SLOT_MASK;
            if (__ballot(!ok) != 0ull) {
                if (!ok) ok = wait_cell(e, lap, false) == DE_V6_SLOT_MASK;
                if (__ballot(!ok) != 0ull) raise(ERR_CELL_BUSY_TIMEOUT);
            }
            if (ok) st_e(e, cell_full(lap, slot));
        }
    }

    DE_DEV void drain_sample(uint32_t live) {
        if (lane_id() != 0) return;
        const unsigned long long t0 = __hip_atomic_load(reinterpret_cast<unsigned long long*>(A.ctl + G_T_EXHAUSTED * DE_V6_CTL_STRIDE), __ATOMIC_RELAXED, __HIP_MEMORY_SCOPE_AGENT);
        const unsigned long long now = __builtin_amdgcn_s_memrealtime();
        if (now < t0) return;
        const unsigned long long bb = (now - t0) / 25000ull + 1ull;
        const uint32_t b = bb < 32ull ? (uint32_t)bb : 32u;
        const uint32_t old = __hip_atomic_fetch_max(cw + 17, b, __ATOMIC_RELAXED, __HIP_MEMORY_SCOPE_WORKGROUP);
        for (uint32_t k = old; k < b; ++k) {
            __hip_atomic_fetch_add(reinterpret_cast<unsigned long long*>(A.ctl + (G_DRAIN + k) * DE_V6_CTL_STRIDE), (unsigned long long)live, __ATOMIC_RELAXED, __HIP_MEMORY_SCOPE_AGENT);
            __hip_atomic_fetch_add(reinterpret_cast<unsigned long long*>(A.ctl + (G_DRAIN + 32u + k) * DE_V6_CTL_STRIDE), 1ull, __ATOMIC_RELAXED, __HIP_MEMORY_SCOPE_AGENT);
        }
    }

    DE_DEV int schedule() {
        uint32_t idle = 0;
        for (;;) {
            const uint32_t l = (uint32_t)lane_id();
            const uint32_t misc = ld_wg(cw + 16 + (l & 7u));
            int ready = 0;
            if (l < (uint32_t)NR) ready = (int)(ld_wg(tail(l)) - ld_wg(head(l)));
            if (!aborted && __builtin_amdgcn_readlane((int)misc, 0) != 0) aborted = true;
            if (aborted) return Q_EXIT;
            primary_left = (uint32_t)__builtin_amdgcn_readlane((int)misc, 3) < A.bands;
            int best_q = -1, best = 0, low_q = -1, low = 0;
#pragma unroll
            for (int q = 0; q < NQ; ++q) {
                const int r = __builtin_amdgcn_readlane(ready, q);
                const bool shallow_flat = q > Q_CLOUD && r < (int)A.flat_min;
                if (!shallow_flat && r > best) { best = r; best_q = q; }
                if (shallow_flat && r > low) { low = r; low_q = q; }
            }
            if (best_q < 0) { best_q = low_q; best = low; }
            if (best_q >= 0 && best < (int)A.enter_min && idle < 4u) best_q = -1;
            const int free_slots = __builtin_amdgcn_readlane(ready, Q_FREE);
            if (STATS && !primary_left) drain_sample((uint32_t)((int)DE_V6_P - free_slots));
            if (A.export_at != 0u && !primary_left) {
                const uint32_t live = DE_V6_P - (uint32_t)free_slots;
                bool exporting = __builtin_amdgcn_readlane((int)misc, 2) != 0;
                if (!exporting && live != 0u && live <= A.export_at) {
                    uint32_t dec = (uint32_t)__builtin_amdgcn_readlane((int)misc, 4);
                    if (dec == 0u) {
                        if (lane_id() == 0) {
                            dec = (A.seq == 0xffffffffu || (int)(__hip_atomic_load(A.issued, __ATOMIC_RELAXED, __HIP_MEMORY_SCOPE_SYSTEM) - A.seq) >= 0) ? 1u : 2u;
                            __hip_atomic_store(cw + 20, dec, __ATOMIC_RELAXED, __HIP_MEMORY_SCOPE_WORKGROUP);
                        }
                        dec = uni(dec);
                    }
                    if (dec == 1u) {
                        if (lane_id() == 0) __hip_atomic_store(cw + 18, 1u, __ATOMIC_RELAXED, __HIP_MEMORY_SCOPE_WORKGROUP);
                        exporting = true;
                    }
                }
                if (exporting) {
                    if (best > 0) return Q_EXPORT;
                    if (free_slots == (int)DE_V6_P) return Q_EXIT;
                    if (++idle > A.idle_limit) { raise(ERR_IDLE_WATCHDOG); return Q_EXIT; }
                    __builtin_amdgcn_s_sleep(8);
                    continue;
                }
            }
            if (primary_left && free_slots >= 64) return Q_PRIMARY;
            if (best_q >= 0) { stat(ST_ENTRIES, 1); return best_q; }
            if (!primary_left && free_slots == (int)DE_V6_P) return Q_EXIT;
            stat(ST_IDLE, 1);
            if (++idle > A.idle_limit) { raise(ERR_IDLE_WATCHDOG); return Q_EXIT; }
            if (idle < 8u) __builtin_amdgcn_s_sleep(2);
            else if (idle < 24u) __builtin_amdgcn_s_sleep(16);
            else if (idle < 64u) __builtin_amdgcn_s_sleep(48);
            else __builtin_amdgcn_s_sleep(100);
        }
    }

    template <int Q, typename Stage, int... TARGETS>
    DE_DEV void run_loop(Stage& st, Targets<TARGETS...>) {
        const int SERVICE = (int)A.svc[Q];
        const uint32_t AREA = A.svc_area[Q];
        uint32_t idle_acc = 0;
        Path p;
        uint32_t slot = 0;
        bool busy = false, fin = false;
        int target = -1;
        bool dry = false;
        uint32_t trips = 0, retry_at = 0;
        regions_begin();
        for (;;) {
            const int nb = __popcll(__ballot(busy));
            const bool may_refill = !dry || trips >= retry_at;
            if (nb == 0 || ((AREA != 0u || 64 - nb >= SERVICE) && (may_refill || __ballot(fin) != 0ull))) {
                idle_acc = 0u;
                tick<R_HEAD>(0ull);
                if (STATS) r_cnt[0]++;
                if (__ballot(fin) != 0ull) {
                    const unsigned long long n_fin = STATS ? (unsigned long long)__popcll(__ballot(fin)) : 0ull;
                    if (fin) { target = st.finish(p); store_rec(rec, slot, p); }
                    tick<R_EPI>(n_fin);
                    release_wg();
                    (push<TARGETS>(slot, fin && target == TARGETS), ...);
                    fin = false;
                    tick<R_PUSH>(n_fin);
                }
                if (may_refill || nb == 0) {
                    dry = false;
                    const unsigned long long m_need = __ballot(!busy);
                    uint32_t first = 0;
                    const uint32_t got = claim(Q, 1u, (uint32_t)__popcll(m_need), &first);
                    if (got == 0u) {
                        dry = true; retry_at = trips + A.retry;
                        tick<R_REFILL>(0ull);
                        if (nb > 0 && ((nb <= (int)A.yield_max && work_elsewhere(Q)) || (A.export_at != 0u && uni(ld_wg(cw + 18)) != 0u))) {
                            if (busy) {
                                st.suspend(p, cold + slot);
                                p.meta |= 0x80000000u;
                                store_rec(rec, slot, p);
                            }
                            release_wg();
                            push<Q>(slot, busy);
                            stat(ST_YIELD, 1); stat(ST_YIELDED, (unsigned long long)nb);
                            busy = false;
                            tick<R_YIELD>((unsigned long long)nb);
                            break;
                        }
                    } else {
                        const uint32_t my = (uint32_t)__popcll(m_need & ((1ull << lane_id()) - 1ull));
                        const bool mine = !busy && my < got;
                        uint32_t s = 0;
                        if (mine) s = take(Q, first + my);
                        if (__ballot(mine && s == DE_V6_EMPTY) != 0ull) { raise(ERR_ENTRY_TIMEOUT); break; }
                        acquire_wg();
                        if (mine) {
                            slot = s; load_rec(rec, slot, p);
                            const bool resumed = (p.meta & 0x80000000u) != 0u;
                            p.meta &= 0x7fffffffu;
                            st.begin(p);
                            if (resumed) st.restore(cold + slot);
                            busy = true;
                        }
                        stat(ST_RECS + Q, got);
                        tick<R_REFILL>((unsigned long long)got);
                    }
                }
                if (__ballot(busy) == 0ull) { if (dry || aborted) break; else continue; }
            }
            const bool was_busy = busy;
            do {
                const unsigned long long n_step = STATS ? (unsigned long long)__popcll(__ballot(busy)) : 0ull;
                if (STATS) { stat(ST_TRIPS + Q, 1); stat(ST_LANETRIPS + Q, n_step); r_cnt[1]++; }
                tick<R_HEAD>(0ull);
                const bool stepping = busy;
                if (busy) {
                    if (st.step(p)) busy = false;
                }
                if constexpr (STATS && Q == Q_CLOUD) cloud_stats(st, stepping);
                tick<R_STEP>(n_step);
                trips++;
                idle_acc += (uint32_t)(64 - __popcll(__ballot(busy)));
            } while (idle_acc < AREA);
            fin = fin || (was_busy && !busy);
        }
        tick<R_HEAD>(0ull);
        regions_end_loop(Q);
    }
    DE_DEV bool work_elsewhere(uint32_t q) {
        int ready = 0;
        const uint32_t l = (uint32_t)lane_id();
        if (l < (uint32_t)NR && l != q) ready = (int)(ld_wg(tail(l)) - ld_wg(head(l)));
        if (l == (uint32_t)Q_FREE && !starters()) ready = 0;
        return __ballot(ready >= (int)A.elsewhere_min) != 0ull;
    }

    template <int Q>
    DE_DEV void export_ring(const Pool& pool) {
        for (;;) {
            uint32_t first = 0;
            const uint32_t n = claim(Q, 1u, 64u, &first);
            if (n == 0u) break;
            const bool active = (uint32_t)lane_id() < n;
            uint32_t slot = 0;
            if (active) slot = take(Q, first + (uint32_t)lane_id());
            if (__ballot(active && slot == DE_V6_EMPTY) != 0ull) { raise(ERR_ENTRY_TIMEOUT); break; }
            acquire_wg();
            uint32_t base = 0;
            if (lane_id() == 0) base = __hip_atomic_fetch_add(A.ctl + (G_POOL + 2u * A.level) * DE_V6_CTL_STRIDE, n, __ATOMIC_RELAXED, __HIP_MEMORY_SCOPE_AGENT);
            base = uni(base);
            if (base + n > A.cap_out) { raise(ERR_POOL_FULL); break; }
            if (active) {
                const uint32_t i = base + (uint32_t)lane_id();
                pool.a[i] = rec[slot]; pool.b[i] = rec[DE_V6_P + slot]; pool.c[i] = rec[2u * DE_V6_P + slot]; pool.d[i] = s_rec2[slot];
                const uint4* cs = reinterpret_cast<const uint4*>(cold + slot);
#pragma unroll
                for (uint32_t k = 0; k < 4u; ++k) pool.cold[(size_t)k * A.cap_out + i] = cs[k];
                pool.q[i] = (uint32_t)Q;
            }
            push<Q_FREE>(slot, active);
        }
    }
    template <int... QS>
    DE_DEV void run_export(Targets<QS...>) {
        const Pool pool(A.pool_out, A.cap_out);
        (export_ring<QS>(pool), ...);
    }
    DE_DEV void run_import() {
        uint32_t first = 0;
        if (claim(Q_FREE, 64u, 64u, &first) == 0u) { stat(ST_CLAIMFAIL, 1); return; }
        uint32_t slot = take(Q_FREE, first + (uint32_t)lane_id());
        if (__ballot(slot == DE_V6_EMPTY) != 0ull) { raise(ERR_ENTRY_TIMEOUT); return; }
        acquire_wg();
        uint32_t w = 0, total = 0;
        if (lane_id() == 0) {
            w = __hip_atomic_fetch_add(A.ctl + (G_POOL + 2u * (A.level - 1u) + 1u) * DE_V6_CTL_STRIDE, 64u, __ATOMIC_RELAXED, __HIP_MEMORY_SCOPE_AGENT);
            total = __hip_atomic_load(A.ctl + (G_POOL + 2u * (A.level - 1u)) * DE_V6_CTL_STRIDE, __ATOMIC_RELAXED, __HIP_MEMORY_SCOPE_AGENT);
        }
        w = uni(w); total = min(uni(total), A.cap_in);
        const uint32_t n = w < total ? min(64u, total - w) : 0u;
        const bool active = (uint32_t)lane_id() < n;
        uint32_t q = 0xffu;
        if (active) {
            const Pool pool(A.pool_in, A.cap_in);
            const uint32_t i = w + (uint32_t)lane_id();
            rec[slot] = pool.a[i]; rec[DE_V6_P + slot] = pool.b[i]; rec[2u * DE_V6_P + slot] = pool.c[i]; s_rec2[slot] = pool.d[i];
            uint4* cd = reinterpret_cast<uint4*>(cold + slot);
#pragma unroll
            for (uint32_t k = 0; k < 4u; ++k) cd[k] = pool.cold[(size_t)k * A.cap_in + i];
            q = pool.q[i];
        }
        stat(ST_RECS + NQ, n);
        release_wg();
        push<Q_ST>(slot, q == (uint32_t)Q_ST); push<Q_GAS>(slot, q == (uint32_t)Q_GAS); push<Q_CLOUD>(slot, q == (uint32_t)Q_CLOUD); push<Q_EVENT>(slot, q == (uint32_t)Q_EVENT);
        push<Q_SURF>(slot, q == (uint32_t)Q_SURF); push<Q_SCFIN>(slot, q == (uint32_t)Q_SCFIN); push<Q_SURFFIN>(slot, q == (uint32_t)Q_SURFFIN);
        push<Q_FREE>(slot, !active);
        if (n < 64u && lane_id() == 0) __hip_atomic_store(cw + 19, 0xffffffffu, __ATOMIC_RELAXED, __HIP_MEMORY_SCOPE_WORKGROUP);
    }

    template <int Q, typename Body, int... TARGETS>
    DE_DEV void run_flat(Body body, Targets<TARGETS...>) {
        regions_begin();
        uint32_t kmin = 1u;
        for (;;) {
            uint32_t first = 0;
            const uint32_t n = claim(Q, kmin, 64u, &first);
            if (n == 0u) break;
            kmin = A.flat_again;
            const bool active = (uint32_t)lane_id() < n;
            uint32_t slot = 0;
            if (active) slot = take(Q, first + (uint32_t)lane_id());
            if (__ballot(active && slot == DE_V6_EMPTY) != 0ull) { raise(ERR_ENTRY_TIMEOUT); break; }
            acquire_wg();
            Path p;
            int target = -2;
            if (active) {
                load_rec(rec, slot, p);
                p.pid = wf::asu(cold[slot].pad0);
            }
            tick<R_PUSH>(0ull);
            if (active) {
                target = body(p, ColdAt{cold + slot});
            }
            tick<R_STEP>((unsigned long long)n);
            if (active && target >= 0) store_rec(rec, slot, p);
            stat(ST_RECS + Q, n);
            if (STATS) { stat(ST_TRIPS + Q, 1); stat(ST_LANETRIPS + Q, n); r_cnt[0]++; }
            release_wg();
            (push<TARGETS>(slot, target == TARGETS), ...);
            push<Q_FREE>(slot, target == -1);
            tick<R_PUSH>(0ull);
        }
        tick<R_PUSH>(0ull);
        regions_end_flat(42 + 4 * (Q - 3));
    }

    DE_DEV void run_primary(const RenderArgs& a, const FrameConsts& fc) {
        regions_begin();
        primary_batch(a, fc);
        regions_end_flat(58);
    }
    DE_DEV void primary_batch(const RenderArgs& a, const FrameConsts& fc) {
        uint32_t first = 0;
        if (claim(Q_FREE, 64u, 64u, &first) == 0u) { stat(ST_CLAIMFAIL, 1); return; }
        uint32_t slot = take(Q_FREE, first + (uint32_t)lane_id());
        if (__ballot(slot == DE_V6_EMPTY) != 0ull) { raise(ERR_ENTRY_TIMEOUT); return; }
        const uint32_t nb = A.bands, spp = (uint32_t)a.spp_count, per = ((uint32_t)a.n_tiles + nb - 1u) / nb;
        uint32_t tries = uni(ld_wg(cw + 19)), w0 = 0u, n = 0u;
        for (;;) {
            if (tries >= nb) {
                primary_left = false;
                const unsigned long long now = __builtin_amdgcn_s_memrealtime();
                if (lane_id() == 0) __hip_atomic_fetch_min(reinterpret_cast<unsigned long long*>(A.ctl + G_T_EXHAUSTED * DE_V6_CTL_STRIDE), now, __ATOMIC_RELAXED, __HIP_MEMORY_SCOPE_AGENT);
                break;
            }
            const uint32_t band = (A.xcd + tries) % nb;
            const uint32_t lo = min(band * per, (uint32_t)a.n_tiles) * 64u * spp, hi = min((band + 1u) * per, (uint32_t)a.n_tiles) * 64u * spp;
            uint32_t w = 0;
            if (lane_id() == 0) w = __hip_atomic_fetch_add(A.ctl + (G_WORKX + band) * DE_V6_CTL_STRIDE, 64u, __ATOMIC_RELAXED, __HIP_MEMORY_SCOPE_AGENT);
            w = uni(w);
            if (w < hi - lo) { w0 = lo + w; n = min(64u, hi - lo - w); break; }
            tries++;
            if (lane_id() == 0) __hip_atomic_fetch_max(cw + 19, tries, __ATOMIC_RELAXED, __HIP_MEMORY_SCOPE_WORKGROUP);
        }
        const uint32_t w = w0 + (uint32_t)lane_id();
        const bool active = (uint32_t)lane_id() < n;
        acquire_wg();
        const float MAX_RAY_DIST = (float)(6371e3 * 10.0);
        Path p;
        int target = -2;
        tick<R_PUSH>(0ull);
        if (active) {
            wf::new_path(a, fc, bs::s_node_val, w, p);
            const float t = wf::sphere_trace<CLAMP>(a, p, fc.land_height_scale, DE_PLANET_R + de_max(fc.land_height_scale, 0.0f) + 8100.0f, MAX_RAY_DIST);
            target = wf::after_sphere_trace(p, t, MAX_RAY_DIST);
            store_rec(rec, slot, p);
            cold[slot].pad0 = wf::asf(p.pid);
        }
        tick<R_STEP>((unsigned long long)n);
        stat(ST_RECS + NQ, n);
        if (STATS) r_cnt[0]++;
        release_wg();
        push<Q_GAS>(slot, target == Q_GAS);
        push<Q_CLOUD>(slot, target == Q_CLOUD);
        push<Q_EVENT>(slot, target == Q_EVENT);
        push<Q_FREE>(slot, !active);
        tick<R_PUSH>(0ull);
    }
};

}


__global__ void v6_init_kernel(uint32_t* ctl, RenderArgs a, RenderArgs* dst) {
    const uint32_t i = blockIdx.x * blockDim.x + threadIdx.x;
    if (i < (uint32_t)bs::G_WORDS) {
        const uint32_t fill = (i == (uint32_t)bs::G_T_START || i == (uint32_t)bs::G_T_EXHAUSTED) ? 0xffffffffu : 0u;
        ctl[i * DE_V6_CTL_STRIDE] = fill; ctl[i * DE_V6_CTL_STRIDE + 1u] = fill;
    }
    if (i == 0u) *dst = a;
}

#define DE_V6_STAGE template <bool CLAMP, bool STATS> static __device__ __attribute__((noinline)) void
DE_V6_STAGE v6_stage_st() {
    using namespace bs;
    Wave<CLAMP, STATS> W = Wave<CLAMP, STATS>::enter();
    const RenderArgs& a = *W.A.ra;
    const FrameConsts& fc = *W.A.fc;
    const float MAX_RAY_DIST = (float)(6371e3 * 10.0);
    StStage<CLAMP> st{a.topo, fc.land_height_scale, DE_PLANET_R + de_max(fc.land_height_scale, 0.0f) + 8100.0f, MAX_RAY_DIST, 0.0f, 0};
    W.template run_loop<Q_ST>(st, Targets<Q_GAS, Q_CLOUD, Q_EVENT, Q_SURFFIN>{});
}
DE_V6_STAGE v6_stage_gas() {
    using namespace bs;
    Wave<CLAMP, STATS> W = Wave<CLAMP, STATS>::enter();
    const RenderArgs& a = *W.A.ra;
    GasStage st{uni_ptr(a.nodes), uni_ptr(a.dens_table)};
    W.template run_loop<Q_GAS>(st, Targets<Q_CLOUD, Q_EVENT, Q_SCFIN, Q_SURFFIN>{});
}
DE_V6_STAGE v6_stage_cloud() {
    using namespace bs;
    Wave<CLAMP, STATS> W = Wave<CLAMP, STATS>::enter();
    const RenderArgs& a = *W.A.ra;
#ifndef DE_NO_CLOUD_BOUND
    CloudStage<CLAMP, true> st{uni_tex(a.clouds), uni_ptr(a.cloud_bound)};
#else
    CloudStage<CLAMP> st{uni_tex(a.clouds)};
#endif
    W.template run_loop<Q_CLOUD>(st, Targets<Q_EVENT, Q_SCFIN, Q_SURFFIN>{});
}
DE_V6_STAGE v6_stage_event() {
    using namespace bs;
    Wave<CLAMP, STATS> W = Wave<CLAMP, STATS>::enter();
    const RenderArgs& a = *W.A.ra;
    const FrameConsts& fc = *W.A.fc;
    W.template run_flat<Q_EVENT>([&](Path& p, const ColdAt& cold) { return wf::event_body<CLAMP>(a, fc, cold, p); }, Targets<Q_GAS, Q_CLOUD, Q_SCFIN, Q_SURF>{});
}
DE_V6_STAGE v6_stage_surf() {
    using namespace bs;
    Wave<CLAMP, STATS> W = Wave<CLAMP, STATS>::enter();
    const RenderArgs& a = *W.A.ra;
    const FrameConsts& fc = *W.A.fc;
    W.template run_flat<Q_SURF>([&](Path& p, const ColdAt& cold) { return wf::surf_body<CLAMP>(a, fc, cold, p); }, Targets<Q_ST>{});
}
DE_V6_STAGE v6_stage_scfin() {
    using namespace bs;
    Wave<CLAMP, STATS> W = Wave<CLAMP, STATS>::enter();
    const RenderArgs& a = *W.A.ra;
    const FrameConsts& fc = *W.A.fc;
    W.template run_flat<Q_SCFIN>([&](Path& p, const ColdAt& cold) { return wf::scfin_body(a, fc, cold, p); }, Targets<Q_ST>{});
}
DE_V6_STAGE v6_stage_surffin() {
    using namespace bs;
    Wave<CLAMP, STATS> W = Wave<CLAMP, STATS>::enter();
    const RenderArgs& a = *W.A.ra;
    W.template run_flat<Q_SURFFIN>([&](Path& p, const ColdAt& cold) { return wf::surffin_body(a, cold, p); }, Targets<Q_ST>{});
}

DE_V6_STAGE v6_stage_export() {
    using namespace bs;
    Wave<CLAMP, STATS> W = Wave<CLAMP, STATS>::enter();
    W.run_export(Targets<Q_ST, Q_GAS, Q_CLOUD, Q_EVENT, Q_SURF, Q_SCFIN, Q_SURFFIN>{});
}
DE_V6_STAGE v6_stage_import() {
    using namespace bs;
    Wave<CLAMP, STATS> W = Wave<CLAMP, STATS>::enter();
    W.run_import();
}
DE_V6_STAGE v6_stage_primary() {
    using namespace bs;
    Wave<CLAMP, STATS> W = Wave<CLAMP, STATS>::enter();
    const RenderArgs& a = *wf::opaque_ptr(W.A.ra);
    const FrameConsts& fc = *wf::opaque_ptr(W.A.fc);
    W.run_primary(a, fc);
}

template <bool CLAMP, bool STATS, bool TAIL>
__global__ void __attribute__((amdgpu_flat_work_group_size(64 * DE_V6_WAVES, 64 * DE_V6_WAVES), amdgpu_waves_per_eu(DE_V6_WPE, DE_V6_WPE)))
v6_kernel(bs::Args A, const FrameConsts* fcp) {
    using namespace bs;
    for (uint32_t i = threadIdx.x; i < NR * DE_V6_CAP; i += blockDim.x) {
        const uint32_t q = i / DE_V6_CAP, k = i % DE_V6_CAP;
        s_rings[i] = (uint16_t)((q == (uint32_t)Q_FREE && k < DE_V6_P) ? cell_full(0u, k) : cell_empty(0u));
    }
    if (threadIdx.x < 32u) s_cw[threadIdx.x] = (threadIdx.x == 8u + (uint32_t)Q_FREE) ? DE_V6_P : 0u;
    if (threadIdx.x < 64u) { s_node_val[threadIdx.x] = A.ra->node_val[threadIdx.x]; s_stats[threadIdx.x] = 0ull; }
    if (threadIdx.x == 0u) {
        Cfg c;
        c.ra = A.ra; c.fc = fcp; c.cold = A.cold + (size_t)blockIdx.x * DE_V6_P; c.ctl = A.ctl; c.status = A.status;
        c.n_items = A.n_items; c.idle_limit = A.idle_limit;
        c.svc[0] = A.svc[0]; c.svc[1] = A.svc[1]; c.svc[2] = A.svc[2];
        c.svc_area[0] = A.svc_area[0]; c.svc_area[1] = A.svc_area[1]; c.svc_area[2] = A.svc_area[2];
        c.yield_max = A.yield_max; c.elsewhere_min = A.elsewhere_min; c.retry = A.retry; c.enter_min = A.enter_min; c.flat_min = A.flat_min; c.flat_again = A.flat_again;
        c.bands = A.bands == 8u ? 8u : 1u;
        c.pool_in = A.pool_in; c.pool_out = A.pool_out; c.level = A.level; c.export_at = A.export_at; c.cap_in = A.cap_in; c.cap_out = A.cap_out; c.issued = A.issued; c.seq = A.seq; c.pad_ = 0u;
        { uint32_t xcc; asm volatile("s_getreg_b32 %0, hwreg(HW_REG_XCC_ID)" : "=s"(xcc)); c.xcd = xcc & 7u; }
        const uint32_t* src = reinterpret_cast<const uint32_t*>(&c);
        for (uint32_t k = 0; k < sizeof(Cfg) / 4u; ++k) s_cfg[k] = src[k];
    }
    __syncthreads();
    if (!TAIL && threadIdx.x == 0u) __hip_atomic_fetch_min(reinterpret_cast<unsigned long long*>(A.ctl + G_T_START * DE_V6_CTL_STRIDE), (unsigned long long)__builtin_amdgcn_s_memrealtime(), __ATOMIC_RELAXED, __HIP_MEMORY_SCOPE_AGENT);
    unsigned long long t_mark = STATS ? __builtin_amdgcn_s_memrealtime() : 0ull;
    for (;;) {
        Wave<CLAMP, STATS> W = Wave<CLAMP, STATS>::enter();
        W.t_mark = t_mark;
        const int s = __builtin_amdgcn_readfirstlane(W.schedule());
        W.template mark<-1>();
        if (s == Q_EXIT) {
            const unsigned long long now = __builtin_amdgcn_s_memrealtime();
            if (lane_id() == 0) __hip_atomic_fetch_max(reinterpret_cast<unsigned long long*>(A.ctl + G_T_END * DE_V6_CTL_STRIDE), now, __ATOMIC_RELAXED, __HIP_MEMORY_SCOPE_AGENT);
            if (STATS) {
                const unsigned long long t0 = __hip_atomic_load(reinterpret_cast<unsigned long long*>(A.ctl + G_T_EXHAUSTED * DE_V6_CTL_STRIDE), __ATOMIC_RELAXED, __HIP_MEMORY_SCOPE_AGENT);
                if (t0 != ~0ull && now > t0) W.stat(ST_DRAIN, now - t0);
            }
            break;
        }
        if (STATS && s < NQ) W.stat(ST_ENTRY_Q + s, 1);
        switch (s) {
        case Q_ST: v6_stage_st<CLAMP, STATS>(); W.template mark<Q_ST>(); break;
        case Q_GAS: v6_stage_gas<CLAMP, STATS>(); W.template mark<Q_GAS>(); break;
        case Q_CLOUD: v6_stage_cloud<CLAMP, STATS>(); W.template mark<Q_CLOUD>(); break;
        case Q_EVENT: v6_stage_event<CLAMP, STATS>(); W.template mark<Q_EVENT>(); break;
        case Q_SURF: v6_stage_surf<CLAMP, STATS>(); W.template mark<Q_SURF>(); break;
        case Q_SCFIN: v6_stage_scfin<CLAMP, STATS>(); W.template mark<Q_SCFIN>(); break;
        case Q_SURFFIN: v6_stage_surffin<CLAMP, STATS>(); W.template mark<Q_SURFFIN>(); break;
        case Q_EXPORT: v6_stage_export<CLAMP, STATS>(); W.template mark<-1>(); break;
        default:
            if (TAIL) v6_stage_import<CLAMP, STATS>(); else v6_stage_primary<CLAMP, STATS>();
            W.template mark<7>();
            break;
        }
        t_mark = W.t_mark;
    }
    if (STATS) {
        __syncthreads();
        if (threadIdx.x < (uint32_t)ST_N && s_stats[threadIdx.x])
            __hip_atomic_fetch_add(reinterpret_cast<unsigned long long*>(A.ctl + (G_STAT0 + threadIdx.x) * DE_V6_CTL_STRIDE), s_stats[threadIdx.x], __ATOMIC_RELAXED, __HIP_MEMORY_SCOPE_AGENT);
    }
}
```

Before: 1479 Msamples/s.

## Add clear-cloud fast-path stage queue routed by cloud bound lookup

Adds a new scheduler queue and stage (Q_CLEAR) that handles short cloud segments whose cloud-bound cell is zero. These segments take a cheap delta-tracking path that only advances the RNG and distance, with no density lookups, and fall back to the full cloud stage if a travel budget is exceeded. Several stages now consult the bound at routing time. To fit the extra ring in LDS, the per-CU record pool shrinks from 1120 to 1088 and the control words are relaid out. The risks are lower in-flight occupancy, extra scheduler overhead, and divergence from the extra queue.

```diff
diff --git a/digital_earth_amd/build.py b/digital_earth_amd/build.py
--- a/digital_earth_amd/build.py
+++ b/digital_earth_amd/build.py
@@ -48,8 +48,9 @@
     return OUT_LEGACY
 
 
-TEST_VARIANTS = (("v6_p64", ["-DDE_V6_P=64u", "-DDE_V6_CAP=65u"]), ("v6_p128", ["-DDE_V6_P=128u", "-DDE_V6_CAP=129u"]), ("v6_cap_p1", ["-DDE_V6_CAP=1121u"]),
-                 ("v6_no_cloud_bound", ["-DDE_NO_CLOUD_BOUND"]))
+TEST_VARIANTS = (("v6_p64", ["-DDE_V6_P=64u", "-DDE_V6_CAP=65u"]), ("v6_p128", ["-DDE_V6_P=128u", "-DDE_V6_CAP=129u"]), ("v6_cap_p1", ["-DDE_V6_CAP=1089u"]),
+                 ("v6_no_cloud_bound", ["-DDE_NO_CLOUD_BOUND"]),
+                 ("v6_clear_budget", ["-DDE_CLOUD_CLEAR_BUDGET=48"]))
 
 
 def build_test_variants(force=False, verbose=False):
diff --git a/digital_earth_amd/csrc/de_context.h b/digital_earth_amd/csrc/de_context.h
--- a/digital_earth_amd/csrc/de_context.h
+++ b/digital_earth_amd/csrc/de_context.h
@@ -157,6 +157,10 @@
     int v6_stats = 0;
     int v6_svc[3] = {24, 24, 20};
     int v6_svc_area[3] = {100, 72, 90};
+#ifndef DE_V6_CLEAR_AREA
+#define DE_V6_CLEAR_AREA 270
+#endif
+    int v6_clear_area = DE_V6_CLEAR_AREA;
     int v6_yield = 56, v6_elsewhere = 48, v6_retry = 6, v6_enter_min = 0, v6_flat_min = 0, v6_flat_again = 32;
     int launch_variant = 2;
     int launch_pipe = 0;
diff --git a/digital_earth_amd/csrc/de_kernels.h b/digital_earth_amd/csrc/de_kernels.h
--- a/digital_earth_amd/csrc/de_kernels.h
+++ b/digital_earth_amd/csrc/de_kernels.h
@@ -85,6 +85,10 @@
 #define DE_CLOUD_BOUND_R 24576u
 #endif
 #define DE_CLOUD_BOUND_BYTES (6u * DE_CLOUD_BOUND_N * DE_CLOUD_BOUND_N)
+#ifndef DE_CLOUD_CLEAR_LEN
+#define DE_CLOUD_CLEAR_LEN 12288.0f
+#endif
+static_assert(DE_CLOUD_CLEAR_LEN <= (float)(DE_CLOUD_BOUND_R / 2u), "a clear segment must fit into half the bound's travel budget");
 DE_DEV uint32_t cloud_bound_cell(float x, float y, float z) {
     const float ax = de_abs(x), ay = de_abs(y), az = de_abs(z);
     float s, t, m;
diff --git a/digital_earth_amd/csrc/de_launch.h b/digital_earth_amd/csrc/de_launch.h
--- a/digital_earth_amd/csrc/de_launch.h
+++ b/digital_earth_amd/csrc/de_launch.h
@@ -223,6 +223,7 @@
     A.n_items = (uint32_t)((size_t)a.n_tiles * 64u * (size_t)a.spp_count);
     A.idle_limit = 1u << 22;
     for (int k = 0; k < 3; ++k) { A.svc[k] = (uint32_t)c->v6_svc[k]; A.svc_area[k] = (uint32_t)c->v6_svc_area[k]; }
+    A.svc[3] = (uint32_t)c->v6_svc[2]; A.svc_area[3] = (uint32_t)c->v6_clear_area;
     A.yield_max = (uint32_t)c->v6_yield; A.elsewhere_min = (uint32_t)c->v6_elsewhere; A.retry = (uint32_t)c->v6_retry; A.enter_min = (uint32_t)c->v6_enter_min; A.flat_min = (uint32_t)c->v6_flat_min; A.flat_again = (uint32_t)(c->v6_flat_again > 0 ? c->v6_flat_again : 1);
     A.bands = c->v6_bands == 8 ? 8u : 1u;
     hipLaunchKernelGGL(v6_init_kernel, dim3(1), dim3(256), 0, stream, S.ctl, a, S.d_args);
diff --git a/digital_earth_amd/csrc/de_stages.h b/digital_earth_amd/csrc/de_stages.h
--- a/digital_earth_amd/csrc/de_stages.h
+++ b/digital_earth_amd/csrc/de_stages.h
@@ -48,6 +48,21 @@
     if (kind == 0) { p.x[0] = t_start; p.x[1] = aux; p.x[2] = X; return Q_EVENT; }
     p.x[0] = aux; p.x[1] = 1.0f; p.x[2] = X;
     return kind == 1 ? Q_SCFIN : Q_SURFFIN;
+}
+enum { Q_CLEAR = NQ };
+DE_DEV uint32_t cloud_first_byte(const Path& p, const uint8_t* bound) {
+    const vec3 C0 = p.P + p.x[0] * p.W;
+    const uint32_t cell = cloud_bound_cell(C0.x, C0.y, C0.z);
+#ifdef __HIP_DEVICE_COMPILE__
+    typedef const __attribute__((address_space(1))) uint8_t* de_gbytes;
+    return (uint32_t)*((de_gbytes)bound + cell);
+#else
+    return (uint32_t)bound[cell];
+#endif
+}
+DE_DEV int cloud_or_clear(const Path& p, const uint8_t* bound) {
+    if (!(p.x[1] - p.x[0] <= DE_CLOUD_CLEAR_LEN)) return Q_CLOUD;
+    return cloud_first_byte(p, bound) == 0u ? (int)Q_CLEAR : (int)Q_CLOUD;
 }
 DE_DEV int after_sphere_trace(Path& p, float t, float max_ray_dist) {
     const int kind = m_kind(p.meta);
@@ -506,3 +521,49 @@
     DE_DEV void suspend(wf::Path& p, wf::Cold* c) const { p.x[0] = t; c->pad1 = trn; c->pad2 = C.x; c->pad3 = C.y; c->pad4 = C.z; }
     DE_DEV void restore(const wf::Cold* c) { trn = c->pad1; C = v3(c->pad2, c->pad3, c->pad4); bnd = 0xffffffffu; }
 };
+
+#ifndef DE_CLOUD_CLEAR_BUDGET
+#define DE_CLOUD_CLEAR_BUDGET DE_CLOUD_BOUND_R
+#endif
+struct ClearStage {
+    static constexpr bool kBound = false;
+    float rmaxc, t, tmax;
+    Rng g;
+    int kind;
+    int32_t budget;
+    bool fallback;
+    DE_DEV void begin(wf::Path& p) {
+        const int sc = wf::m_sc(p.meta);
+        rmaxc = (sc > 9) ? (1.0f / (0.02f * DE_CLOUDS_DENSITY)) : (1.0f / (DE_CLOUDS_EXTINCT * DE_CLOUDS_DENSITY));
+        kind = wf::m_kind(p.meta);
+        t = p.x[0]; tmax = p.x[1];
+        g = p.rng;
+        budget = (int32_t)(DE_CLOUD_CLEAR_BUDGET); fallback = false;
+    }
+    DE_DEV bool step(wf::Path&) {
+        const float neg_log = -de_log_unit(rng_next(g));
+        const float t_step = neg_log * rmaxc;
+        t += t_step;
+        if (t >= tmax) return true;
+        Rng g2 = g;
+        (void)rng_next(g2);
+        const bool delta = kind == 0;
+        g.s0 = delta ? g2.s0 : g.s0; g.s1 = delta ? g2.s1 : g.s1;
+        budget -= (int32_t)((uint32_t)t_step + 1u);
+        fallback = budget < 0;
+        return fallback | !(t < tmax);
+    }
+    DE_DEV int finish(wf::Path& p) {
+        if (fallback) return wf::Q_CLOUD;
+        const float aux = p.x[2], X = p.x[3];
+        p.rng.s0 = g.s0; p.rng.s1 = g.s1;
+        if (kind == 0) {
+            p.x[0] = t; p.x[1] = aux; p.x[2] = X;
+            return wf::Q_EVENT;
+        }
+        p.x[0] = aux; p.x[1] = 1.0f; p.x[2] = X;
+        return (kind == 1) ? wf::Q_SCFIN : wf::Q_SURFFIN;
+    }
+    DE_DEV void suspend(wf::Path&, wf::Cold* c) const { c->pad1 = t; c->pad2 = wf::asf(g.s0); c->pad3 = wf::asf(g.s1); c->pad4 = wf::asf((uint32_t)budget); }
+    DE_DEV void restore(const wf::Cold* c) { t = c->pad1; g.s0 = wf::asu(c->pad2); g.s1 = wf::asu(c->pad3); budget = (int32_t)wf::asu(c->pad4); }
+};
diff --git a/digital_earth_amd/csrc/render_kernel_v6.hip b/digital_earth_amd/csrc/render_kernel_v6.hip
--- a/digital_earth_amd/csrc/render_kernel_v6.hip
+++ b/digital_earth_amd/csrc/render_kernel_v6.hip
@@ -6,7 +6,15 @@
 using wf::NQ;
 using wf::Q_ST; using wf::Q_GAS; using wf::Q_CLOUD; using wf::Q_EVENT; using wf::Q_SURF; using wf::Q_SCFIN; using wf::Q_SURFFIN;
 
-enum { Q_FREE = NQ, NR = NQ + 1, Q_PRIMARY = NQ + 1, Q_EXIT = NQ + 2, Q_EXPORT = NQ + 3 };
+#if defined(DE_NO_CLOUD_BOUND) || defined(DE_NO_CLOUD_CLEAR)
+#define DE_V6_CLEAR 0
+#define DE_V6_CLEAR_T
+#else
+#define DE_V6_CLEAR 1
+#define DE_V6_CLEAR_T , Q_CLEAR
+#endif
+using wf::Q_CLEAR;
+enum { NQS = NQ + DE_V6_CLEAR, Q_FREE = NQS, NR = NQS + 1, Q_PRIMARY = NQS + 1, Q_EXIT = NQS + 2, Q_EXPORT = NQS + 3 };
 #ifndef DE_V6_WAVES
 #define DE_V6_WAVES 12
 #endif
@@ -17,10 +25,14 @@
 #define DE_V6_WPE 6
 #endif
 #ifndef DE_V6_P
+#if DE_V6_CLEAR
+#define DE_V6_P 1088u
+#else
 #define DE_V6_P 1120u
 #endif
+#endif
 #ifndef DE_V6_CAP
-#define DE_V6_CAP 1128u
+#define DE_V6_CAP (DE_V6_P + 8u)
 #endif
 #define DE_V6_EMPTY 0xffffu
 #define DE_V6_SLOT_MASK 0x7ffu
@@ -30,7 +42,12 @@
 #define DE_V6_CTL_STRIDE 32u
 enum { G_WORK = 0, G_T_START = 1, G_T_EXHAUSTED = 2, G_T_END = 3, G_STAT0 = 8, G_STAT2 = 8 + 64, G_WORKX = 8 + 64 + 64, G_DRAIN = 8 + 64 + 64 + 8, G_POOL = 8 + 64 + 64 + 8 + 64, G_WORDS = 8 + 64 + 64 + 8 + 64 + 8 };
 enum { R_STEP = 0, R_EPI, R_PUSH, R_REFILL, R_YIELD, R_HEAD, R_N };
-enum { ST_RECS = 0, ST_CYC = 8, ST_IDLE = 16, ST_ENTRIES = 17, ST_CLAIMFAIL = 18, ST_SCHED = 19, ST_YIELD = 20, ST_YIELDED = 21, ST_DRAIN = 22, ST_CLOUD_EXACT = 23, ST_ENTRY_Q = 24, ST_CLOUD_NOEXACT = 31, ST_TRIPS = 32, ST_CLOUD_LOOKUPS = 39, ST_LANETRIPS = 40, ST_N = 48 };
+enum { ST_RECS = 0, ST_CYC = 8, ST_IDLE = 16, ST_ENTRIES = 17, ST_CLAIMFAIL = 18, ST_SCHED = 19, ST_YIELD = 20, ST_YIELDED = 21, ST_DRAIN = 22, ST_CLOUD_EXACT = 23, ST_ENTRY_Q = 24, ST_CLOUD_NOEXACT = 31, ST_TRIPS = 32, ST_CLOUD_LOOKUPS = 39, ST_LANETRIPS = 40,
+       ST_CLEAR_RECS = 48, ST_CLEAR_CYC = 49, ST_CLEAR_ENTRIES = 50, ST_CLEAR_TRIPS = 51, ST_CLEAR_LANETRIPS = 52, ST_CC_RECS = 53, ST_CC_CLEAR = 54, ST_CC_B0 = 55, ST_CC_HIST = 56, ST_N = 64 };
+constexpr int st_of(int base, int q, int clear_word) { return q == (int)wf::NQ ? clear_word : base + q; }
+enum { CW_TAIL = 16, CW_MISC = 32, CW_WORDS = 48 };
+static_assert(NR <= CW_TAIL, "one head and one tail word per ring");
+constexpr int svc_of(int q) { return q == (int)wf::NQ ? 3 : q; }
 enum { ERR_ENTRY_TIMEOUT = 1, ERR_CELL_BUSY_TIMEOUT = 2, ERR_IDLE_WATCHDOG = 3, ERR_POOL_FULL = 4 };
 DE_DEV uint32_t cell_empty(uint32_t lap) { return (lap << 11) | DE_V6_SLOT_MASK; }
 DE_DEV uint32_t cell_full(uint32_t lap, uint32_t slot) { return (lap << 11) | slot; }
@@ -43,8 +60,8 @@
     uint32_t* status;
     uint32_t n_items;
     uint32_t idle_limit;
-    uint32_t svc[3];
-    uint32_t svc_area[3];
+    uint32_t svc[4];
+    uint32_t svc_area[4];
     uint32_t yield_max;
     uint32_t elsewhere_min;
     uint32_t retry;
@@ -74,8 +91,8 @@
     uint32_t* ctl;
     uint32_t* status;
     uint32_t n_items, idle_limit;
-    uint32_t svc[3];
-    uint32_t svc_area[3];
+    uint32_t svc[4];
+    uint32_t svc_area[4];
     uint32_t yield_max, elsewhere_min, retry, enter_min;
     uint32_t flat_min, flat_again;
     uint32_t bands, xcd;
@@ -87,8 +104,8 @@
 
 __shared__ uint4 s_rec[3u * DE_V6_P];
 __shared__ uint2 s_rec2[DE_V6_P];
-__shared__ uint16_t s_rings[(NQ + 1) * DE_V6_CAP];
-__shared__ uint32_t s_cw[32];
+__shared__ uint16_t s_rings[NR * DE_V6_CAP];
+__shared__ uint32_t s_cw[CW_WORDS];
 __shared__ float s_node_val[64];
 __shared__ unsigned long long s_stats[64];
 __shared__ uint32_t s_cfg[40];
@@ -148,6 +165,7 @@
     uint16_t* rings;
     uint32_t* cw;
     wf::Cold* cold;
+    const uint8_t* bound;
     unsigned long long* s_st;
     bool primary_left, aborted;
     unsigned long long t_mark;
@@ -185,7 +203,7 @@
         uint32_t* dst = reinterpret_cast<uint32_t*>(&W.A);
 #pragma unroll
         for (uint32_t k = 0; k < sizeof(Cfg) / 4u; ++k) dst[k] = uni(s_cfg[k]);
-        W.rec = s_rec; W.rings = s_rings; W.cw = s_cw; W.cold = W.A.cold; W.s_st = s_stats;
+        W.rec = s_rec; W.rings = s_rings; W.cw = s_cw; W.cold = W.A.cold; W.s_st = s_stats; W.bound = nullptr;
         W.primary_left = true; W.aborted = false; W.t_mark = 0ull;
         return W;
     }
@@ -204,20 +222,20 @@
     DE_DEV void mark() {
         if (!STATS) return;
         const unsigned long long t = __builtin_amdgcn_s_memrealtime();
-        stat(STAGE >= 0 ? ST_CYC + STAGE : ST_SCHED, t - t_mark);
+        stat(STAGE == 64 ? (int)ST_CLEAR_CYC : (STAGE >= 0 ? ST_CYC + STAGE : (int)ST_SCHED), t - t_mark);
         t_mark = t;
     }
     DE_DEV uint32_t* head(uint32_t q) const { return cw + q; }
-    DE_DEV uint32_t* tail(uint32_t q) const { return cw + 8u + q; }
+    DE_DEV uint32_t* tail(uint32_t q) const { return cw + (uint32_t)CW_TAIL + q; }
     DE_DEV void raise(uint32_t code) {
         if (lane_id() == 0) {
-            __hip_atomic_store(cw + 16, code, __ATOMIC_RELAXED, __HIP_MEMORY_SCOPE_WORKGROUP);
+            __hip_atomic_store(cw + CW_MISC, code, __ATOMIC_RELAXED, __HIP_MEMORY_SCOPE_WORKGROUP);
             __hip_atomic_store(A.status, code, __ATOMIC_RELAXED, __HIP_MEMORY_SCOPE_SYSTEM);
         }
         aborted = true;
     }
 
-    DE_DEV bool starters() { primary_left = uni(ld_wg(cw + 19)) < A.bands; return primary_left; }
+    DE_DEV bool starters() { primary_left = uni(ld_wg(cw + CW_MISC + 3)) < A.bands; return primary_left; }
 
     DE_DEV uint32_t claim(uint32_t q, uint32_t kmin, uint32_t kmax, uint32_t* first) {
         uint32_t got = 0, hh = 0;
@@ -278,6 +296,20 @@
         }
     }
 
+    DE_DEV int route(const Path& p, bool to_cloud, int target) {
+        if (to_cloud) target = wf::cloud_or_clear(p, bound);
+        if (STATS) {
+            const float len = p.x[1] - p.x[0];
+            const bool b0 = to_cloud && (target == Q_CLEAR || (!(len <= DE_CLOUD_CLEAR_LEN) && wf::cloud_first_byte(p, bound) == 0u));
+            stat(ST_CC_RECS, (unsigned long long)__popcll(__ballot(to_cloud)));
+            stat(ST_CC_CLEAR, (unsigned long long)__popcll(__ballot(to_cloud && target == Q_CLEAR)));
+            stat(ST_CC_B0, (unsigned long long)__popcll(__ballot(b0)));
+#pragma unroll
+            for (int k = 0; k < 8; ++k) stat(ST_CC_HIST + k, (unsigned long long)__popcll(__ballot(b0 && (k == 7 ? !(len < 14000.0f) : (len >= 2000.0f * (float)k && len < 2000.0f * (float)(k + 1))))));
+        }
+        return target;
+    }
+
     DE_DEV void drain_sample(uint32_t live) {
         if (lane_id() != 0) return;
         const unsigned long long t0 = __hip_atomic_load(reinterpret_cast<unsigned long long*>(A.ctl + G_T_EXHAUSTED * DE_V6_CTL_STRIDE), __ATOMIC_RELAXED, __HIP_MEMORY_SCOPE_AGENT);
@@ -285,7 +317,7 @@
         if (now < t0) return;
         const unsigned long long bb = (now - t0) / 25000ull + 1ull;
         const uint32_t b = bb < 32ull ? (uint32_t)bb : 32u;
-        const uint32_t old = __hip_atomic_fetch_max(cw + 17, b, __ATOMIC_RELAXED, __HIP_MEMORY_SCOPE_WORKGROUP);
+        const uint32_t old = __hip_atomic_fetch_max(cw + CW_MISC + 1, b, __ATOMIC_RELAXED, __HIP_MEMORY_SCOPE_WORKGROUP);
         for (uint32_t k = old; k < b; ++k) {
             __hip_atomic_fetch_add(reinterpret_cast<unsigned long long*>(A.ctl + (G_DRAIN + k) * DE_V6_CTL_STRIDE), (unsigned long long)live, __ATOMIC_RELAXED, __HIP_MEMORY_SCOPE_AGENT);
             __hip_atomic_fetch_add(reinterpret_cast<unsigned long long*>(A.ctl + (G_DRAIN + 32u + k) * DE_V6_CTL_STRIDE), 1ull, __ATOMIC_RELAXED, __HIP_MEMORY_SCOPE_AGENT);
@@ -296,7 +328,7 @@
         uint32_t idle = 0;
         for (;;) {
             const uint32_t l = (uint32_t)lane_id();
-            const uint32_t misc = ld_wg(cw + 16 + (l & 7u));
+            const uint32_t misc = ld_wg(cw + CW_MISC + (l & 7u));
             int ready = 0;
             if (l < (uint32_t)NR) ready = (int)(ld_wg(tail(l)) - ld_wg(head(l)));
             if (!aborted && __builtin_amdgcn_readlane((int)misc, 0) != 0) aborted = true;
@@ -304,9 +336,9 @@
             primary_left = (uint32_t)__builtin_amdgcn_readlane((int)misc, 3) < A.bands;
             int best_q = -1, best = 0, low_q = -1, low = 0;
 #pragma unroll
-            for (int q = 0; q < NQ; ++q) {
+            for (int q = 0; q < NQS; ++q) {
                 const int r = __builtin_amdgcn_readlane(ready, q);
-                const bool shallow_flat = q > Q_CLOUD && r < (int)A.flat_min;
+                const bool shallow_flat = q > Q_CLOUD && q < NQ && r < (int)A.flat_min;
                 if (!shallow_flat && r > best) { best = r; best_q = q; }
                 if (shallow_flat && r > low) { low = r; low_q = q; }
             }
@@ -322,12 +354,12 @@
                     if (dec == 0u) {
                         if (lane_id() == 0) {
                             dec = (A.seq == 0xffffffffu || (int)(__hip_atomic_load(A.issued, __ATOMIC_RELAXED, __HIP_MEMORY_SCOPE_SYSTEM) - A.seq) >= 0) ? 1u : 2u;
-                            __hip_atomic_store(cw + 20, dec, __ATOMIC_RELAXED, __HIP_MEMORY_SCOPE_WORKGROUP);
+                            __hip_atomic_store(cw + CW_MISC + 4, dec, __ATOMIC_RELAXED, __HIP_MEMORY_SCOPE_WORKGROUP);
                         }
                         dec = uni(dec);
                     }
                     if (dec == 1u) {
-                        if (lane_id() == 0) __hip_atomic_store(cw + 18, 1u, __ATOMIC_RELAXED, __HIP_MEMORY_SCOPE_WORKGROUP);
+                        if (lane_id() == 0) __hip_atomic_store(cw + CW_MISC + 2, 1u, __ATOMIC_RELAXED, __HIP_MEMORY_SCOPE_WORKGROUP);
                         exporting = true;
                     }
                 }
@@ -353,8 +385,9 @@
 
     template <int Q, typename Stage, int... TARGETS>
     DE_DEV void run_loop(Stage& st, Targets<TARGETS...>) {
-        const int SERVICE = (int)A.svc[Q];
-        const uint32_t AREA = A.svc_area[Q];
+        const int SERVICE = (int)A.svc[svc_of(Q)];
+        const uint32_t AREA = A.svc_area[svc_of(Q)];
+        constexpr bool ROUTE = DE_V6_CLEAR && ((TARGETS == (int)Q_CLEAR) || ...);
         uint32_t idle_acc = 0;
         Path p;
         uint32_t slot = 0;
@@ -373,6 +406,7 @@
                 if (__ballot(fin) != 0ull) {
                     const unsigned long long n_fin = STATS ? (unsigned long long)__popcll(__ballot(fin)) : 0ull;
                     if (fin) { target = st.finish(p); store_rec(rec, slot, p); }
+                    if constexpr (ROUTE) target = route(p, fin && target == Q_CLOUD, target);
                     tick<R_EPI>(n_fin);
                     release_wg();
                     (push<TARGETS>(slot, fin && target == TARGETS), ...);
@@ -387,7 +421,7 @@
                     if (got == 0u) {
                         dry = true; retry_at = trips + A.retry;
                         tick<R_REFILL>(0ull);
-                        if (nb > 0 && ((nb <= (int)A.yield_max && work_elsewhere(Q)) || (A.export_at != 0u && uni(ld_wg(cw + 18)) != 0u))) {
+                        if (nb > 0 && ((nb <= (int)A.yield_max && work_elsewhere(Q)) || (A.export_at != 0u && uni(ld_wg(cw + CW_MISC + 2)) != 0u))) {
                             if (busy) {
                                 st.suspend(p, cold + slot);
                                 p.meta |= 0x80000000u;
@@ -415,7 +449,7 @@
                             if (resumed) st.restore(cold + slot);
                             busy = true;
                         }
-                        stat(ST_RECS + Q, got);
+                        stat(st_of(ST_RECS, Q, ST_CLEAR_RECS), got);
                         tick<R_REFILL>((unsigned long long)got);
                     }
                 }
@@ -424,7 +458,7 @@
             const bool was_busy = busy;
             do {
                 const unsigned long long n_step = STATS ? (unsigned long long)__popcll(__ballot(busy)) : 0ull;
-                if (STATS) { stat(ST_TRIPS + Q, 1); stat(ST_LANETRIPS + Q, n_step); r_cnt[1]++; }
+                if (STATS) { stat(st_of(ST_TRIPS, Q, ST_CLEAR_TRIPS), 1); stat(st_of(ST_LANETRIPS, Q, ST_CLEAR_LANETRIPS), n_step); r_cnt[1]++; }
                 tick<R_HEAD>(0ull);
                 const bool stepping = busy;
                 if (busy) {
@@ -438,7 +472,7 @@
             fin = fin || (was_busy && !busy);
         }
         tick<R_HEAD>(0ull);
-        regions_end_loop(Q);
+        if constexpr (Q < 3) regions_end_loop(Q);
     }
     DE_DEV bool work_elsewhere(uint32_t q) {
         int ready = 0;
@@ -507,8 +541,9 @@
         release_wg();
         push<Q_ST>(slot, q == (uint32_t)Q_ST); push<Q_GAS>(slot, q == (uint32_t)Q_GAS); push<Q_CLOUD>(slot, q == (uint32_t)Q_CLOUD); push<Q_EVENT>(slot, q == (uint32_t)Q_EVENT);
         push<Q_SURF>(slot, q == (uint32_t)Q_SURF); push<Q_SCFIN>(slot, q == (uint32_t)Q_SCFIN); push<Q_SURFFIN>(slot, q == (uint32_t)Q_SURFFIN);
+        if constexpr (DE_V6_CLEAR) push<Q_CLEAR>(slot, q == (uint32_t)Q_CLEAR);
         push<Q_FREE>(slot, !active);
-        if (n < 64u && lane_id() == 0) __hip_atomic_store(cw + 19, 0xffffffffu, __ATOMIC_RELAXED, __HIP_MEMORY_SCOPE_WORKGROUP);
+        if (n < 64u && lane_id() == 0) __hip_atomic_store(cw + CW_MISC + 3, 0xffffffffu, __ATOMIC_RELAXED, __HIP_MEMORY_SCOPE_WORKGROUP);
     }
 
     template <int Q, typename Body, int... TARGETS>
@@ -535,6 +570,7 @@
             if (active) {
                 target = body(p, ColdAt{cold + slot});
             }
+            if constexpr (DE_V6_CLEAR && ((TARGETS == (int)Q_CLEAR) || ...)) target = route(p, active && target == Q_CLOUD, target);
             tick<R_STEP>((unsigned long long)n);
             if (active && target >= 0) store_rec(rec, slot, p);
             stat(ST_RECS + Q, n);
@@ -559,7 +595,7 @@
         uint32_t slot = take(Q_FREE, first + (uint32_t)lane_id());
         if (__ballot(slot == DE_V6_EMPTY) != 0ull) { raise(ERR_ENTRY_TIMEOUT); return; }
         const uint32_t nb = A.bands, spp = (uint32_t)a.spp_count, per = ((uint32_t)a.n_tiles + nb - 1u) / nb;
-        uint32_t tries = uni(ld_wg(cw + 19)), w0 = 0u, n = 0u;
+        uint32_t tries = uni(ld_wg(cw + CW_MISC + 3)), w0 = 0u, n = 0u;
         for (;;) {
             if (tries >= nb) {
                 primary_left = false;
@@ -574,7 +610,7 @@
             w = uni(w);
             if (w < hi - lo) { w0 = lo + w; n = min(64u, hi - lo - w); break; }
             tries++;
-            if (lane_id() == 0) __hip_atomic_fetch_max(cw + 19, tries, __ATOMIC_RELAXED, __HIP_MEMORY_SCOPE_WORKGROUP);
+            if (lane_id() == 0) __hip_atomic_fetch_max(cw + CW_MISC + 3, tries, __ATOMIC_RELAXED, __HIP_MEMORY_SCOPE_WORKGROUP);
         }
         const uint32_t w = w0 + (uint32_t)lane_id();
         const bool active = (uint32_t)lane_id() < n;
@@ -590,12 +626,14 @@
             store_rec(rec, slot, p);
             cold[slot].pad0 = wf::asf(p.pid);
         }
+        if constexpr (DE_V6_CLEAR) target = route(p, active && target == Q_CLOUD, target);
         tick<R_STEP>((unsigned long long)n);
         stat(ST_RECS + NQ, n);
         if (STATS) r_cnt[0]++;
         release_wg();
         push<Q_GAS>(slot, target == Q_GAS);
         push<Q_CLOUD>(slot, target == Q_CLOUD);
+        if constexpr (DE_V6_CLEAR) push<Q_CLEAR>(slot, target == Q_CLEAR);
         push<Q_EVENT>(slot, target == Q_EVENT);
         push<Q_FREE>(slot, !active);
         tick<R_PUSH>(0ull);
@@ -622,14 +660,16 @@
     const FrameConsts& fc = *W.A.fc;
     const float MAX_RAY_DIST = (float)(6371e3 * 10.0);
     StStage<CLAMP> st{a.topo, fc.land_height_scale, DE_PLANET_R + de_max(fc.land_height_scale, 0.0f) + 8100.0f, MAX_RAY_DIST, 0.0f, 0};
-    W.template run_loop<Q_ST>(st, Targets<Q_GAS, Q_CLOUD, Q_EVENT, Q_SURFFIN>{});
+    W.bound = uni_ptr(a.cloud_bound);
+    W.template run_loop<Q_ST>(st, Targets<Q_GAS, Q_CLOUD, Q_EVENT, Q_SURFFIN DE_V6_CLEAR_T>{});
 }
 DE_V6_STAGE v6_stage_gas() {
     using namespace bs;
     Wave<CLAMP, STATS> W = Wave<CLAMP, STATS>::enter();
     const RenderArgs& a = *W.A.ra;
     GasStage st{uni_ptr(a.nodes), uni_ptr(a.dens_table)};
-    W.template run_loop<Q_GAS>(st, Targets<Q_CLOUD, Q_EVENT, Q_SCFIN, Q_SURFFIN>{});
+    W.bound = uni_ptr(a.cloud_bound);
+    W.template run_loop<Q_GAS>(st, Targets<Q_CLOUD, Q_EVENT, Q_SCFIN, Q_SURFFIN DE_V6_CLEAR_T>{});
 }
 DE_V6_STAGE v6_stage_cloud() {
     using namespace bs;
@@ -642,12 +682,21 @@
 #endif
     W.template run_loop<Q_CLOUD>(st, Targets<Q_EVENT, Q_SCFIN, Q_SURFFIN>{});
 }
+#if DE_V6_CLEAR
+DE_V6_STAGE v6_stage_clear() {
+    using namespace bs;
+    Wave<CLAMP, STATS> W = Wave<CLAMP, STATS>::enter();
+    ClearStage st;
+    W.template run_loop<Q_CLEAR>(st, Targets<Q_CLOUD, Q_EVENT, Q_SCFIN, Q_SURFFIN>{});
+}
+#endif
 DE_V6_STAGE v6_stage_event() {
     using namespace bs;
     Wave<CLAMP, STATS> W = Wave<CLAMP, STATS>::enter();
     const RenderArgs& a = *W.A.ra;
     const FrameConsts& fc = *W.A.fc;
-    W.template run_flat<Q_EVENT>([&](Path& p, const ColdAt& cold) { return wf::event_body<CLAMP>(a, fc, cold, p); }, Targets<Q_GAS, Q_CLOUD, Q_SCFIN, Q_SURF>{});
+    W.bound = uni_ptr(a.cloud_bound);
+    W.template run_flat<Q_EVENT>([&](Path& p, const ColdAt& cold) { return wf::event_body<CLAMP>(a, fc, cold, p); }, Targets<Q_GAS, Q_CLOUD, Q_SCFIN, Q_SURF DE_V6_CLEAR_T>{});
 }
 DE_V6_STAGE v6_stage_surf() {
     using namespace bs;
@@ -673,7 +722,7 @@
 DE_V6_STAGE v6_stage_export() {
     using namespace bs;
     Wave<CLAMP, STATS> W = Wave<CLAMP, STATS>::enter();
-    W.run_export(Targets<Q_ST, Q_GAS, Q_CLOUD, Q_EVENT, Q_SURF, Q_SCFIN, Q_SURFFIN>{});
+    W.run_export(Targets<Q_ST, Q_GAS, Q_CLOUD, Q_EVENT, Q_SURF, Q_SCFIN, Q_SURFFIN DE_V6_CLEAR_T>{});
 }
 DE_V6_STAGE v6_stage_import() {
     using namespace bs;
@@ -685,6 +734,7 @@
     Wave<CLAMP, STATS> W = Wave<CLAMP, STATS>::enter();
     const RenderArgs& a = *wf::opaque_ptr(W.A.ra);
     const FrameConsts& fc = *wf::opaque_ptr(W.A.fc);
+    W.bound = uni_ptr(a.cloud_bound);
     W.run_primary(a, fc);
 }
 
@@ -696,14 +746,13 @@
         const uint32_t q = i / DE_V6_CAP, k = i % DE_V6_CAP;
         s_rings[i] = (uint16_t)((q == (uint32_t)Q_FREE && k < DE_V6_P) ? cell_full(0u, k) : cell_empty(0u));
     }
-    if (threadIdx.x < 32u) s_cw[threadIdx.x] = (threadIdx.x == 8u + (uint32_t)Q_FREE) ? DE_V6_P : 0u;
+    if (threadIdx.x < (uint32_t)CW_WORDS) s_cw[threadIdx.x] = (threadIdx.x == (uint32_t)CW_TAIL + (uint32_t)Q_FREE) ? DE_V6_P : 0u;
     if (threadIdx.x < 64u) { s_node_val[threadIdx.x] = A.ra->node_val[threadIdx.x]; s_stats[threadIdx.x] = 0ull; }
     if (threadIdx.x == 0u) {
         Cfg c;
         c.ra = A.ra; c.fc = fcp; c.cold = A.cold + (size_t)blockIdx.x * DE_V6_P; c.ctl = A.ctl; c.status = A.status;
         c.n_items = A.n_items; c.idle_limit = A.idle_limit;
-        c.svc[0] = A.svc[0]; c.svc[1] = A.svc[1]; c.svc[2] = A.svc[2];
-        c.svc_area[0] = A.svc_area[0]; c.svc_area[1] = A.svc_area[1]; c.svc_area[2] = A.svc_area[2];
+        for (int k = 0; k < 4; ++k) { c.svc[k] = A.svc[k]; c.svc_area[k] = A.svc_area[k]; }
         c.yield_max = A.yield_max; c.elsewhere_min = A.elsewhere_min; c.retry = A.retry; c.enter_min = A.enter_min; c.flat_min = A.flat_min; c.flat_again = A.flat_again;
         c.bands = A.bands == 8u ? 8u : 1u;
         c.pool_in = A.pool_in; c.pool_out = A.pool_out; c.level = A.level; c.export_at = A.export_at; c.cap_in = A.cap_in; c.cap_out = A.cap_out; c.issued = A.issued; c.seq = A.seq; c.pad_ = 0u;
@@ -728,7 +777,7 @@
             }
             break;
         }
-        if (STATS && s < NQ) W.stat(ST_ENTRY_Q + s, 1);
+        if (STATS && s < NQS) W.stat(s == (int)NQ ? (int)ST_CLEAR_ENTRIES : ST_ENTRY_Q + s, 1);
         switch (s) {
         case Q_ST: v6_stage_st<CLAMP, STATS>(); W.template mark<Q_ST>(); break;
         case Q_GAS: v6_stage_gas<CLAMP, STATS>(); W.template mark<Q_GAS>(); break;
@@ -737,6 +786,9 @@
         case Q_SURF: v6_stage_surf<CLAMP, STATS>(); W.template mark<Q_SURF>(); break;
         case Q_SCFIN: v6_stage_scfin<CLAMP, STATS>(); W.template mark<Q_SCFIN>(); break;
         case Q_SURFFIN: v6_stage_surffin<CLAMP, STATS>(); W.template mark<Q_SURFFIN>(); break;
+#if DE_V6_CLEAR
+        case Q_CLEAR: v6_stage_clear<CLAMP, STATS>(); W.template mark<64>(); break;
+#endif
         case Q_EXPORT: v6_stage_export<CLAMP, STATS>(); W.template mark<-1>(); break;
         default:
             if (TAIL) v6_stage_import<CLAMP, STATS>(); else v6_stage_primary<CLAMP, STATS>();
```

Result: no change. 1480 Msamples/s, median of 2 (+0.1%).
